# cselab/smarties

Measured on AMD Instinct MI355X. Metric: learner transitions/sec, VRACER batch=256 over 1M replay, higher is better.
Workload: dtype f32; 1 GPU; VRACER learner update, synthetic replay 5000 episodes x 200 transitions = 1M (state_dim 17, act_dim 6 bounded), 2x256 SoftSign MLP (72976 padded fp32 params), global batch 256 split over 1 replica(s), replay split likewise, device-side mt19937 sampler; global_batch=256, replay_transitions=1000000, parallelism=dp1, exchange=single replica

## Files before the change

smarties_amd/csrc/fused.hip:

```cpp
#include "tail_dev.h"

namespace hl {

#define FLDR 258
#define FLDS 34
#define FMAXK4 8
#ifndef FUSED_NT
#define FUSED_NT 512
#endif
#ifndef FUSED_CHAINW
#define FUSED_CHAINW 8
#endif
#ifndef FUSED_PRE_LATE
#define FUSED_PRE_LATE 1
#endif
#ifndef FUSED_H1_PRE
#define FUSED_H1_PRE 1
#endif
#ifndef FUSED_ARGS_FIRST
#define FUSED_ARGS_FIRST 1
#endif
#define FTLD 17

#if defined(HL_FSTAMPS)
// ... 13 lines not shown
#define FEND(i) do { } while (0)
#endif

#ifdef HL_DEV
#define FVARIANT_STOP(n) do { if (a.variant == (n)) return; } while (0)
#else
#define FVARIANT_STOP(n) do { } while (0)
#endif

__host__ __device__ inline int fusedR2Floats(int dSp, int H) { return dSp * (H + 16); }
__host__ __device__ inline int fusedR3Floats(int H) { const int a = H * 16, b = 16 * FLDR; return a > b ? a : b; }
__host__ __device__ inline size_t fusedLdsBytes(int dS, int H) {
  const int dSp = (dS + 3) & ~3;
  const size_t fl = (size_t)16 * FLDR + fusedR2Floats(dSp, H) + fusedR3Floats(H) + (size_t)H * 8  + 16 * FLDS +
                    2048  + 3 * (size_t)H  + 512  + 128  + 2 * (16 * FTLD + 16)  + 32  + 4 ;
  const size_t bytes = fl * 4;
  return bytes > TAIL_LDS_BYTES ? bytes : TAIL_LDS_BYTES;
}

template <int NK, class FA, class FB>
__device__ __forceinline__ f32x4 waveMma(FA fa, FB fb) {
  float av[NK], bv[NK];
#pragma unroll
  for (int s = 0; s < NK; ++s) { av[s] = fa(s); bv[s] = fb(s); }
  f32x4 acc0 = {0.f, 0.f, 0.f, 0.f}, acc1 = {0.f, 0.f, 0.f, 0.f};
#pragma unroll
  for (int s = 0; s < NK; ++s) {
    if (s & 1) acc1 = __builtin_amdgcn_mfma_f32_16x16x4f32(av[s], bv[s], acc1, 0, 0, 0);
    else acc0 = __builtin_amdgcn_mfma_f32_16x16x4f32(av[s], bv[s], acc0, 0, 0, 0);
  }
  return acc0 + acc1;
}

template <int NQ, int NTL, bool TILE_A, class FS, class FT>
__device__ __forceinline__ void h1Steps(f32x4* acc, FS fs, FT ft) {
  float sv[NQ], tv[NQ][NTL];
#pragma unroll
  for (int s = 0; s < NQ; ++s) {
    sv[s] = fs(s);
#pragma unroll
    for (int t = 0; t < NTL; ++t) tv[s][t] = ft(s, t);
  }
  __builtin_amdgcn_sched_barrier(0);
#pragma unroll
  for (int s = 0; s < NQ; ++s) {
#pragma unroll
    for (int t = 0; t < NTL; ++t) {
      if constexpr (TILE_A) acc[t] = __builtin_amdgcn_mfma_f32_16x16x4f32(tv[s][t], sv[s], acc[t], 0, 0, 0);
      else acc[t] = __builtin_amdgcn_mfma_f32_16x16x4f32(sv[s], tv[s][t], acc[t], 0, 0, 0);
    }
  }
}
template <int NTL, bool TILE_A, class FS, class FT>
__device__ __forceinline__ void h1Product(int nk4, f32x4* acc, FS fs, FT ft) {
  switch (nk4) {
    case 1: h1Steps<1, NTL, TILE_A>(acc, fs, ft); break;
    case 2: h1Steps<2, NTL, TILE_A>(acc, fs, ft); break;
    case 3: h1Steps<3, NTL, TILE_A>(acc, fs, ft); break;
    case 4: h1Steps<4, NTL, TILE_A>(acc, fs, ft); break;
    case 5: h1Steps<5, NTL, TILE_A>(acc, fs, ft); break;
    case 6: h1Steps<6, NTL, TILE_A>(acc, fs, ft); break;
    case 7: h1Steps<7, NTL, TILE_A>(acc, fs, ft); break;
    case 8: h1Steps<8, NTL, TILE_A>(acc, fs, ft); break;
    default: break;
  }
}

template <int NP> __device__ __forceinline__ float redSum(const float* red, int tid) {
  if constexpr (NP == 8) return ((red[tid] + red[256 + tid]) + (red[512 + tid] + red[768 + tid])) + ((red[1024 + tid] + red[1280 + tid]) + (red[1536 + tid] + red[1792 + tid]));
  else return (red[tid] + red[256 + tid]) + (red[512 + tid] + red[768 + tid]);
}

template <int N> __device__ __forceinline__ float treeSum(const float* v) {
  if constexpr (N == 1) return v[0];
  else return treeSum<N / 2>(v) + treeSum<N / 2>(v + N / 2);
}

template <int H, int CF, int NT>
__global__ __launch_bounds__(NT, NT / 128) void fused_fwd_head_dx_kernel(FusedArgs a, ExtraArgs extra) {
  extern __shared__ __attribute__((aligned(16))) unsigned char smem[];
  if (blockIdx.x < 8) {
    if (threadIdx.x >= 256) return;
    if (blockIdx.x == 0) { if (extra.role == 1) { samplePhases(extra.samp, extra.phases, smem); FEND(22); } }
    else if (blockIdx.x == 1 && (a.deferBeta || extra.post.mode == POST_ENCODE)) { farBetaPhase(extra.post, smem); if (threadIdx.x == 0) a.sc->dbgT[23] = wall_clock64(); }
    else if (extra.role == 1 && (extra.phases & PH_PUBLISH)) gatherHelper(extra.samp, blockIdx.x - 1, 7, smem);
    return;
  }
  constexpr int HT = H / 16, H4 = H / 4, LDW0 = H + 16;
  constexpr int NW = NT / 64;
  constexpr int KWAVES = (H / 4 >= NW) ? NW : 4;
  constexpr int KW = H / KWAVES;
  constexpr int NK = KW / 4;
  constexpr int TPW = HT >= NW ? HT / NW : 1;
  constexpr int QP = (16 * H4 + NT - 1) / NT;
  constexpr int QC = (H * 4 + NT - 1) / NT;
  constexpr int QO = (H * 2 + NT - 1) / NT;
  constexpr int Q0 = (32 * H4 + NT - 1) / NT;
  constexpr int QS = 512 / NT;
  constexpr bool CHAIN = (NW == 8 && H >= 64);
  constexpr int CW = (FUSED_CHAINW == 8 && H >= 128) ? 8 : 4;
  constexpr int CT = CHAIN ? H / (16 * CW) : 1;
  constexpr int CTID = CW == 8 ? 0 : 256;
  constexpr int TLD = CHAIN ? FTLD : 16;
  constexpr int TY1 = 16 * FTLD + 16;
#if defined(HL_FSTAMPS)
  if (threadIdx.x == 0 && blockIdx.x == 8 + 8) a.sc->dbgT[31] = wall_clock64();
#endif
#ifdef HL_TAIL_STAMPS
  if (threadIdx.x == 0 && blockIdx.x == 8 + 8) a.sc->dbgT[31] = wall_clock64();
#endif
#ifdef HL_STEP_STAMPS
  if (threadIdx.x == 0 && blockIdx.x == 8 + 8) a.sc->dbgStep[a.sc->nGradSteps & 63] = wall_clock64();
#endif
  const DevScalars* sc = a.sc;
  const float* W = a.W; const float* X0 = a.X0; unsigned* panelCtr = a.panelCtr;
  long long iW0 = a.indW0, iW1 = a.indW1, iWo = a.indWo, iB0 = a.indB0, iB1 = a.indB1, iWr = a.indWr, iBr = a.indBr, iBo = a.indBo, iBp = a.indBp;
  int ldW0 = a.ldW0, ldW1 = a.ldW1, ldX0 = a.ldX0, dSa = a.dS, Ba = a.B, parity = a.parity;
#if FUSED_ARGS_FIRST
  asm volatile("" :: "s"(W), "s"(iW0), "s"(iW1), "s"(iWo), "s"(iB0), "s"(iB1), "s"(iWr), "s"(iBr), "s"(iBo), "s"(iBp),
               "s"(X0), "s"(panelCtr), "s"(sc), "s"(ldW0), "s"(ldW1), "s"(ldX0), "s"(dSa), "s"(Ba), "s"(parity),
               "s"(a.bt.nextSrc), "s"(a.bt.slot), "s"(a.bt.eid));
#endif
  const int dS = dSa, dSp = (dS + 3) & ~3, B = Ba, dA = a.dA, nDense = a.nDense;
  const int func = __builtin_amdgcn_readfirstlane(a.func);
  int resN = a.resN, ldA0 = a.ldA0, ldA1 = a.ldA1;
  float* gR2 = a.R2; float* gX2 = a.X2; float* gD2 = a.D2; float* gDres2 = a.Dres2;
#define FUSED_PIN_ARGS() do { asm volatile("" : "+v"(resN), "+v"(ldA0), "+v"(ldA1)); asm volatile("" : "+v"(gR2), "+v"(gX2), "+v"(gD2), "+v"(gDres2)); } while (0)
#if !FUSED_ARGS_FIRST
  FUSED_PIN_ARGS();
#endif
  const int bid = blockIdx.x - 8, xcd = bid & 7, gi = bid >> 3;
  const int panel = (gi / HT) * 8 + xcd, n = gi % HT;
  const int m0 = panel * 16, n0 = n * 16;
  int nRows = B;
  if (m0 + 16 > B) { nRows = sc->nRows[parity]; if (m0 >= nRows) return; }
  FSTAMP(0);

  float* sY1 = reinterpret_cast<float*>(smem);
  float* sR2 = sY1 + 16 * FLDR;
  float* sR3 = sR2 + fusedR2Floats(dSp, H);
  float* sWo = sR3 + fusedR3Floats(H);
  float* sS = sWo + H * 8;
  float* red = sS + 16 * FLDS;
  float* sB0 = red + 2048;
  float* sWr = sB0 + H;
  float* sBr = sWr + H;
  double* sO = reinterpret_cast<double*>(sBr + H);
  float* sDo = reinterpret_cast<float*>(sO + 256);
  float* sT = sDo + 128;
  float* sBo = sT + 2 * (16 * FTLD + 16);
  float* sBp = sBo + 16;
  double* sBeta = reinterpret_cast<double*>(sBp + 16);

  const int tid = threadIdx.x, lane = tid & 63;
  __builtin_assume(tid >= 0 && tid < NT);
  const int wave = __builtin_amdgcn_readfirstlane(tid >> 6);
  const int li = lane & 15, lc = lane >> 4;
  const bool eth = tid < 256;
  const int em = (tid >> 4) & 15, en = tid & 15;
  const float* W0 = W + iW0; const float* W1 = W + iW1; const float* Wo = W + iWo;

  const int row = m0 + em;
  const bool rowValid = eth && row < nRows, isNext = rowValid && row >= B;
  int bSrc = 0; long long slot = 0;
  if (rowValid) { bSrc = isNext ? a.bt.nextSrc[row - B] : row; slot = a.bt.slot[bSrc]; }
  int eidv = 0;
  if (rowValid && !isNext) eidv = a.bt.eid[row];
  float sv[QS];
#pragma unroll
  for (int q = 0; q < QS; ++q) {
    const int idx = tid + NT * q, r = idx >> 5, c = idx & 31;
    sv[q] = (c < dS && m0 + r < nRows) ? X0[(size_t)(m0 + r) * ldX0 + c] : 0.f;
  }
  const f32x4 z4 = {0.f, 0.f, 0.f, 0.f};
  f32x4 w0v[Q0], w1c[QC], w1r[QP], wov[QO];
  const int nW0 = dSp * H4;
#pragma unroll
  for (int q = 0; q < Q0; ++q) {
    const int f = tid + NT * q, k = f / H4, c4 = f % H4;
    w0v[q] = *reinterpret_cast<const f32x4*>(W0 + (size_t)(k < dS ? k : dS - 1) * ldW0 + 4 * c4);
  }
#pragma unroll
  for (int q = 0; q < QC; ++q) {
    const int f = tid + NT * q; w1c[q] = z4;
    if (f < H * 4) { const int k = f >> 2, c = n0 + (f & 3) * 4; w1c[q] = *reinterpret_cast<const f32x4*>(W1 + (size_t)k * ldW1 + c); }
  }
#pragma unroll
  for (int q = 0; q < QO; ++q) { const int f = tid + NT * q; wov[q] = f < H * 2 ? *reinterpret_cast<const f32x4*>(Wo + (size_t)f * 4) : z4; }
  const float b0v = tid < H ? W[iB0 + tid] : 0.f;
  const float wrv = tid < H ? W[iWr + tid] : 0.f, brv = tid < H ? W[iBr + tid] : 0.f;
  const float b1e = eth ? W[iB1 + n0 + en] : 0.f;
  const float bov = tid < nDense ? W[iBo + tid] : 0.f, bpv = tid < dA ? W[iBp + tid] : 0.f;
  double beta = sc->beta; const double Cmax = sc->Cmax, Cinv = sc->Cinv;
  const long long betaWant = sc->nGradSteps;
  unsigned ctr0 = 0;
  if constexpr (HT > 1) ctr0 = __hip_atomic_load(panelCtr + panel * 32, __ATOMIC_RELAXED, __HIP_MEMORY_SCOPE_AGENT);
#if FUSED_ARGS_FIRST
  FUSED_PIN_ARGS();
#endif
#pragma unroll
  for (int q = 0; q < QS; ++q) { const int idx = tid + NT * q, r = idx >> 5, c = idx & 31; sS[r * FLDS + c] = sv[q]; }
#pragma unroll
  for (int q = 0; q < Q0; ++q) {
    const int f = tid + NT * q;
    if (f < nW0) { const int k = f / H4, c4 = f % H4; *reinterpret_cast<f32x4*>(sR2 + k * LDW0 + 4 * c4) = w0v[q]; }
  }
#pragma unroll
  for (int q = 0; q < QC; ++q) { const int f = tid + NT * q; if (f < H * 4) *reinterpret_cast<f32x4*>(sR3 + (size_t)f * 4) = w1c[q]; }
#pragma unroll
  for (int q = 0; q < QO; ++q) { const int f = tid + NT * q; if (f < H * 2) *reinterpret_cast<f32x4*>(sWo + (size_t)f * 4) = wov[q]; }
  if (tid < H) { sB0[tid] = b0v; sWr[tid] = wrv; sBr[tid] = brv; }
  if (tid < 16) { sBo[tid] = bov; sBp[tid] = bpv; }
  __syncthreads();
  FSTAMP(1);
  FVARIANT_STOP(1);
#pragma unroll
  for (int q = 0; q < QP; ++q) {
    const int f = tid + NT * q; w1r[q] = z4;
    if (f < 16 * H4) { const int r = f / H4, c4 = f % H4; w1r[q] = *reinterpret_cast<const f32x4*>(W1 + (size_t)(n0 + r) * a.ldW1 + 4 * c4); }
  }
  const bool aggOwner = ((em & (HT - 1)) == n) && rowValid && !isNext && en < AGG_N;

  double act = 0, bMean = 0, bStd = 1; float misc = 0.f;
  if (rowValid && !isNext && en < dA) {
    act = a.rp.A[(size_t)slot * dA + en];
    bMean = a.rp.MU[(size_t)slot * 2 * dA + en]; bStd = a.rp.MU[(size_t)slot * 2 * dA + dA + en];
  }
  if (rowValid) {
    const float* arr = nullptr; long long sl = slot;
    if (!isNext) arr = en == 0 ? a.rp.RET : en == 1 ? a.rp.DQ : en == 2 ? a.rp.DKL : en == 3 ? a.rp.IMPW : en == 4 ? a.rp.V : en == 5 ? a.rp.ADV : nullptr;
    else { arr = en == 6 ? a.rp.V : en == 7 ? a.rp.ADV : nullptr; sl = slot + 1; }
    if (arr) misc = arr[sl];
  }

  float aggv = 0.f;
  if constexpr (CHAIN) {
    asm volatile("" : "+v"(eidv));
    if (aggOwner) aggv = en < AGG_USED ? a.rp.epAgg[(size_t)eidv * AGG_N + en] : (en == AGG_LEN ? (float)a.rp.epN[eidv] : 0.f);
  }

  const bool live = rowValid && !isNext;
  const double MAXM = 8.31776613503286;
  double stdev = 1, invStd = 1, dPos = 0, bInv = 1, invVarMu = 1, u2 = 0, lq = 0, CmuCpi = 1;
  bool bnd = false;
  auto headPrecompute = [&]() {
    asm volatile("" : "+v"(act), "+v"(bMean), "+v"(bStd));
    if (live && en < dA) {
      bnd = ((a.boundedMask >> en) & 1ull) != 0;
      const double pp = (double)sBp[en];
      const double rt = sqrt(1 + pp * pp);
      stdev = (pp + rt) / 2; invStd = 1 / stdev; dPos = (1 + pp / rt) / 2;
      bInv = 1 / bStd; invVarMu = 1 / (bStd * bStd);
      u2 = (act - bMean) * bInv;
      const double qq = stdev * bInv;
      lq = log(qq); CmuCpi = qq * qq;
    }
  };

  float x1o = 0.f, y1o = 0.f;
  if constexpr (!CHAIN) {
  if (wave < HT) {
    f32x4 acc[TPW];
#pragma unroll
    for (int t = 0; t < TPW; ++t) acc[t] = z4;
    const int nk4 = dSp >> 2;
    float bb[TPW];
#pragma unroll
    for (int t = 0; t < TPW; ++t) bb[t] = sB0[(wave + NW * t) * 16 + li];
#if FUSED_H1_PRE
    h1Product<TPW, false>(nk4, acc, [&](int s) { return sS[li * FLDS + 4 * s + lc]; },
                          [&](int s, int t) { return sR2[(4 * s + lc) * LDW0 + (wave + NW * t) * 16 + li]; });
#else
    float av = sS[li * FLDS + lc], bv[TPW];
#pragma unroll
    for (int t = 0; t < TPW; ++t) bv[t] = sR2[lc * LDW0 + (wave + NW * t) * 16 + li];
    for (int s = 0; s < nk4; ++s) {
      const int kn = s + 1 < nk4 ? 4 * (s + 1) + lc : lc;
      const float avn = sS[li * FLDS + kn];
      float bvn[TPW];
#pragma unroll
      for (int t = 0; t < TPW; ++t) bvn[t] = sR2[kn * LDW0 + (wave + NW * t) * 16 + li];
#pragma unroll
      for (int t = 0; t < TPW; ++t) acc[t] = __builtin_amdgcn_mfma_f32_16x16x4f32(av, bv[t], acc[t], 0, 0, 0);
      av = avn;
#pragma unroll
      for (int t = 0; t < TPW; ++t) bv[t] = bvn[t];
    }
#endif
    FSTAMP(14);
    dispatchFunc<CF>(func, [&](auto F) {
      constexpr int FN = decltype(F)::value;
#pragma unroll
      for (int t = 0; t < TPW; ++t) {
        const int nt = wave + NW * t;
        const int c = nt * 16 + li;
#pragma unroll
        for (int r = 0; r < 4; ++r) {
          const int i = lc * 4 + r;
          const float x = acc[t][r] + bb[t];
          sY1[i * FLDR + c] = actEvalT<FN>(x);
          if (nt == n) sT[i * 16 + li] = x;
        }
      }
    });
  }
  FSTAMP(15);
  __syncthreads();
  x1o = sT[em * 16 + en]; y1o = sY1[em * FLDR + n0 + en];
  FSTAMP(2);
  FVARIANT_STOP(2);
  if (eth && row < B) a.Y1[(size_t)row * ldA0 + n0 + en] = y1o;
  asm volatile("" : "+v"(eidv));
  if (aggOwner) aggv = en < AGG_USED ? a.rp.epAgg[(size_t)eidv * AGG_N + en] : (en == AGG_LEN ? (float)a.rp.epN[eidv] : 0.f);
  }
  constexpr bool SPLITW = (NW == 8 && H >= 16);
  constexpr int XW = CHAIN ? CW : (SPLITW ? 4 : KWAVES);
  constexpr int XKW = H / XW, XNK = XKW / 4;

  if constexpr (CHAIN) {
    const int cw = CW == 8 ? wave : wave - 4;
    if (cw >= 0) {
      const int cb = cw * XKW;
      const int pc = (li >> 2) + 4 * (li & 3);
      float w1b[CT][4];
#pragma unroll
      for (int t = 0; t < CT; ++t) {
#pragma unroll
        for (int r = 0; r < 4; ++r) w1b[t][r] = sR3[(cb + 16 * t + 4 * r + lc) * 16 + li];
      }
      f32x4 acc[CT];
#pragma unroll
      for (int t = 0; t < CT; ++t) acc[t] = z4;
      const int nk4 = dSp >> 2;
      float bb[CT][4];
#pragma unroll
      for (int t = 0; t < CT; ++t) {
#pragma unroll
        for (int r = 0; r < 4; ++r) bb[t][r] = sB0[cb + 16 * t + 4 * r + lc];
      }
#if FUSED_H1_PRE
      h1Product<CT, true>(nk4, acc, [&](int s) { return sS[li * FLDS + 4 * s + lc]; },
                          [&](int s, int t) { return sR2[(4 * s + lc) * LDW0 + cb + 16 * t + pc]; });
#else
      float bv = sS[li * FLDS + lc], av[CT];
#pragma unroll
      for (int t = 0; t < CT; ++t) av[t] = sR2[lc * LDW0 + cb + 16 * t + pc];
      for (int s = 0; s < nk4; ++s) {
        const int kn = s + 1 < nk4 ? 4 * (s + 1) + lc : lc;
        const float bvn = sS[li * FLDS + kn];
        float avn[CT];
#pragma unroll
        for (int t = 0; t < CT; ++t) avn[t] = sR2[kn * LDW0 + cb + 16 * t + pc];
#pragma unroll
        for (int t = 0; t < CT; ++t) acc[t] = __builtin_amdgcn_mfma_f32_16x16x4f32(av[t], bv, acc[t], 0, 0, 0);
        bv = bvn;
#pragma unroll
        for (int t = 0; t < CT; ++t) av[t] = avn[t];
      }
#endif
      FSTAMPT(CTID, 14);
      dispatchFunc<CF>(func, [&](auto F) {
        constexpr int FN = decltype(F)::value;
#pragma unroll
        for (int t = 0; t < CT; ++t) {
          const bool own = cb + 16 * t == n0;
#pragma unroll
          for (int r = 0; r < 4; ++r) {
            const float x = acc[t][r] + bb[t][r], y = actEvalT<FN>(x);
            acc[t][r] = y;
            if (own) { sT[li * TLD + 4 * r + lc] = x; sT[TY1 + li * TLD + 4 * r + lc] = y; }
          }
        }
      });
      FSTAMPT(CTID, 15);
      f32x4 xa0 = z4, xa1 = z4;
#pragma unroll
      for (int t = 0; t < CT; ++t) {
#pragma unroll
        for (int r = 0; r < 4; ++r) {
          if (r & 1) xa1 = __builtin_amdgcn_mfma_f32_16x16x4f32(acc[t][r], w1b[t][r], xa1, 0, 0, 0);
          else xa0 = __builtin_amdgcn_mfma_f32_16x16x4f32(acc[t][r], w1b[t][r], xa0, 0, 0, 0);
        }
      }
      const f32x4 xacc = xa0 + xa1;
#pragma unroll
      for (int r = 0; r < 4; ++r) red[cw * 256 + (lc * 4 + r) * 16 + li] = xacc[r];
      FSTAMPT(CTID, 16);
      if (CW == 8 && !FUSED_PRE_LATE) headPrecompute();
    } else if (!FUSED_PRE_LATE) headPrecompute();
    FSTAMP(2);
    FVARIANT_STOP(2);
  } else {
    const int xw = SPLITW ? wave - 4 : wave;
    if (xw >= 0 && xw < XW) {
      const int k0 = xw * XKW + lc;
      const f32x4 acc = waveMma<XNK>([&](int s) { return sY1[li * FLDR + k0 + 4 * s]; }, [&](int s) { return sR3[(k0 + 4 * s) * 16 + li]; });
// ... 187 lines not shown
    const double g0 = far ? 0.0 : Ver * beta * scaleVdiff(O0);
    const double coef = A_RET * fmin(Cmax, RHO);
    if (live && en < dA) {
      const double dMean = mean - bMean;
      const double penalM = -1 * (dMean * invVarMu);
      const double penalS = dPos * -1 * ((invVarMu - invStd * invStd) * stdev);
      double polM = 0, polS = 0;
      if (!far) {
        if (bnd) {
          const double dLogPdMean = (act - mean) * invStd * invStd;
          const double m = mean > MAXM ? MAXM : (mean < -MAXM ? -MAXM : mean);
          const double u = (act - m) * invStd;
          polS = dPos * coef * ((u * u - 1) * invStd);
          if (mean >= MAXM && coef * dLogPdMean > 0) polM = 0;
          else if (mean <= -MAXM && coef * dLogPdMean < 0) polM = 0;
          else polM = coef * dLogPdMean;
        } else {
          const double u = (act - mean) * invStd;
          polM = coef * (u * invStd);
          polS = dPos * coef * ((u * u - 1) * invStd);
        }
      }
      const double gM = beta * polM + (1 - beta) * penalM;
      const double gS = beta * polS + (1 - beta) * penalS;
      gMf = (float)gM;
      if (writer) {
        a.bt.gParam[(size_t)bSrc * dA + en] = (float)gS;
        a.bt.G[(size_t)bSrc * a.nOut + 1 + en] = (double)gMf;
        a.bt.G[(size_t)bSrc * a.nOut + nDense + en] = (double)(float)gS;
      }
    }
    if (live) g0f = (float)g0;
    const float gPrev = rowRorF<1>(gMf);
    if (en < 8) sDo[em * 8 + en] = en == 0 ? g0f : (en <= dA ? gPrev : 0.f);
    if (live && writer) {
      const float oDQ = rowRorF<15>(misc), oDKL = rowRorF<14>(misc), oW = rowRorF<13>(misc);
      const float oV = rowRorF<12>(misc), oADV = rowRorF<11>(misc);
      if (en == 0) {
        a.bt.pEid[bSrc] = a.bt.eid[bSrc]; a.bt.pNextOf[bSrc] = a.bt.nextOf[bSrc];
        a.bt.G[(size_t)bSrc * a.nOut] = (double)g0f;
        a.bt.rho[bSrc] = RHO; a.bt.dkl[bSrc] = DKL; a.bt.far[bSrc] = far ? 1 : 0;
        const float E = (float)dQ, D = (float)DKL, Wn = (float)RHO, Vf = (float)V;
        a.bt.oldDQ[bSrc] = oDQ; a.bt.oldDKL[bSrc] = oDKL; a.bt.oldW[bSrc] = oW; a.bt.oldV[bSrc] = oV; a.bt.oldADV[bSrc] = oADV;
        a.bt.newDQ[bSrc] = E; a.bt.newDKL[bSrc] = D; a.bt.newW[bSrc] = Wn; a.bt.newV[bSrc] = Vf;
        a.rp.DQ[slot] = E; a.rp.DKL[slot] = D; a.rp.IMPW[slot] = Wn; a.rp.V[slot] = Vf; a.rp.ADV[slot] = 0.f;
        a.bt.dq[bSrc] = (double)E;
      }
      if (en < nDense) a.bt.O[(size_t)row * a.nOut + en] = (double)Oen;
      if (en < dA) a.bt.O[(size_t)row * a.nOut + nDense + en] = (double)sBp[en];
    }
  }
  if (NW != 8) stageF2();
  __syncthreads();
  FSTAMP(10);
  FVARIANT_STOP(7);
  if (eth && writer && row < B && en < nDense) a.dOut[(size_t)row * a.ldDo + en] = sDo[em * 8 + en];

  auto deltaY3 = [&](int rowL, int c) {
    const f32x4 wa = *reinterpret_cast<const f32x4*>(sWo + c * 8), wb = *reinterpret_cast<const f32x4*>(sWo + c * 8 + 4);
    const f32x4 da = *reinterpret_cast<const f32x4*>(sDo + rowL * 8), db = *reinterpret_cast<const f32x4*>(sDo + rowL * 8 + 4);
    float s = wa[0] * da[0];
    s = fmaf(wa[1], da[1], s); s = fmaf(wa[2], da[2], s); s = fmaf(wa[3], da[3], s);
    s = fmaf(wb[0], db[0], s); s = fmaf(wb[1], db[1], s); s = fmaf(wb[2], db[2], s); s = fmaf(wb[3], db[3], s);
    return s;
  };
  float dy3own = 0.f;
  if (eth && rowValid) {
    const int c = n0 + en;
    dy3own = deltaY3(em, c);
    if (row < B) { gDres2[(size_t)row * ldA1 + c] = dy3own; gD2[(size_t)row * ldA1 + c] = dy3own * sF2[em * FLDR + c]; }
  }
  FSTAMP(11);
  FVARIANT_STOP(8);

  if (wave < KWAVES) {
    const int k0 = wave * KW + lc;
    const f32x4 acc = waveMma<NK>([&](int s) { const int c = k0 + 4 * s; return deltaY3(li, c) * sF2[li * FLDR + c]; },
                                  [&](int s) { return sBx[li * FLDR + k0 + 4 * s]; });
#pragma unroll
    for (int r = 0; r < 4; ++r) red[wave * 256 + (lc * 4 + r) * 16 + li] = acc[r];
  }
  __syncthreads();
  FSTAMP(12);
  if (((em & (HT - 1)) == n) && rowValid && !isNext && en < AGG_N) a.bt.aggIn[(size_t)bSrc * AGG_N + en] = aggv;
  if (eth && row < B) {
    const float v = redSum<KWAVES>(red, tid);
    float dres = v;
    if (n0 + en < resN) dres += dy3own * sWr[n0 + en];
    a.Dres1[(size_t)row * ldA0 + n0 + en] = dres;
    float f1 = 1.f;
    dispatchFunc<CF>(func, [&](auto F) { f1 = actDiffT<decltype(F)::value>(x1o, y1o); });
    a.D1[(size_t)row * ldA0 + n0 + en] = dres * f1;
  }
  FSTAMP(13);
  FEND(m0 + 16 > a.B ? 21 : 20);
}

template <int H, int CF>
static hipError_t launchFusedT(const FusedArgs& a, int maxRows, const ExtraArgs& ex, hipStream_t s) {
  const int HT = H / 16, panels = (maxRows + 15) / 16, pg = (panels + 7) / 8;
  const size_t lds = fusedLdsBytes(a.dS, H);
  { hipError_t e = ensureDynLds(reinterpret_cast<const void*>(fused_fwd_head_dx_kernel<H, CF, FUSED_NT>), lds); if (e != hipSuccess) return e; }
  hipLaunchKernelGGL((fused_fwd_head_dx_kernel<H, CF, FUSED_NT>), dim3(8 + 8 * HT * pg), dim3(FUSED_NT), lds, s, a, ex);
  return hipGetLastError();
}
template <int H>
static hipError_t launchFusedH(const FusedArgs& a, int maxRows, const ExtraArgs& ex, hipStream_t s) {
  if (a.func == HL_FUNC_SOFTSIGN) return launchFusedT<H, HL_FUNC_SOFTSIGN>(a, maxRows, ex, s);
  if (a.func == HL_FUNC_TANH) return launchFusedT<H, HL_FUNC_TANH>(a, maxRows, ex, s);
  return launchFusedT<H, -1>(a, maxRows, ex, s);
}

hipError_t launch_fused(const FusedArgs& a, int maxRows, const ExtraArgs* extra, hipStream_t s) {
  ExtraArgs ex{}; if (extra) ex = *extra;
  switch (a.H) {
    case 16: return launchFusedH<16>(a, maxRows, ex, s);
    case 32: return launchFusedH<32>(a, maxRows, ex, s);
    case 64: return launchFusedH<64>(a, maxRows, ex, s);
    case 128: return launchFusedH<128>(a, maxRows, ex, s);
    case 256: return launchFusedH<256>(a, maxRows, ex, s);
    default: return hipErrorInvalidValue;
  }
}

size_t fused_lds_bytes(int dS, int H) { return fusedLdsBytes(dS, H); }
int fused_threads() { return FUSED_NT; }

__global__ void xcc_probe_kernel(int* out) {
  extern __shared__ __attribute__((aligned(16))) unsigned char probeSmem[];
  if (threadIdx.x == 0) out[blockIdx.x] = (int)(__builtin_amdgcn_s_getreg((4 - 1) << 11 | 0 << 6 | 20) & 15);
}
hipError_t launch_xcc_probe(int nBlocks, int nThreads, size_t ldsBytes, int* out, hipStream_t s) {
  { hipError_t e = ensureDynLds(reinterpret_cast<const void*>(xcc_probe_kernel), ldsBytes); if (e != hipSuccess) return e; }
  hipLaunchKernelGGL(xcc_probe_kernel, dim3(nBlocks), dim3(nThreads), ldsBytes, s, out);
  return hipGetLastError();
}

}
```

smarties_amd/csrc/fusedw.hip:

```cpp
#include "head_rows.h"

namespace hl {

#define WLDR 258
constexpr int FW_NT = 512;
constexpr int FW_MAXNT = 5;

#ifdef HL_PANEL_STAMPS
#define WSTMP(i) do { if (threadIdx.x == 0 && panel == 0 && n == 1) scw->dbgT[i] = wall_clock64(); } while (0)
#else
#define WSTMP(i) do { } while (0)
#endif

struct FwGeo { int dSp, LS, NTo, LD, LO; size_t oR2, oR3, oWo, oS, oRed, oVec, oO, oXo, oDelta, oMisc, oAct, oBeta, oT, oY4, oF3, oBx2, oW2c, oVec2, total; };
__host__ __device__ inline FwGeo fwGeo(int dS, int H, int nDense, int nOut, int ldWo, int nAdv, int nLH = 2) {
  FwGeo g;
  g.dSp = (dS + 3) & ~3; g.LS = g.dSp + 2;
  g.NTo = (nDense + 15) / 16; g.LD = g.NTo * 16 + 6; g.LO = nOut | 1;
  size_t o = (size_t)16 * WLDR * 4;
  g.oR2 = o; { size_t a = (size_t)g.dSp * 16 * 4, b = (size_t)16 * WLDR * 4, c = nAdv ? (size_t)2 * 16 * 64 * 8 : 0; if (b > a) a = b; if (c > a) a = c; o += a; }
  g.oR3 = o; { size_t a = (size_t)H * 16 * 4, b = (size_t)16 * WLDR * 4; o += a > b ? a : b; }
  g.oWo = o; o += (size_t)H * ldWo * 4;
  g.oS = o; o += (size_t)16 * g.LS * 4;
  g.oRed = o; o += (size_t)8 * g.NTo * 256 * 4;
  g.oVec = o; o += (size_t)3 * H * 4;
  g.oO = (o + 7) & ~(size_t)7; o = g.oO + (size_t)16 * g.LO * 8;
  g.oXo = o; o += (size_t)16 * g.LD * 4;
  g.oDelta = o; o += (size_t)16 * g.LD * 4;
  g.oMisc = o; o += 16 * 8 * 4;
  g.oAct = (o + 7) & ~(size_t)7; o = g.oAct + 16 * 8;
  g.oBeta = o; o += 16;
  g.oT = o; o += 256 * 4;
  g.oY4 = g.oF3 = g.oBx2 = g.oW2c = g.oVec2 = o;
  if (nLH == 3) {
    g.oY4 = o; o += (size_t)16 * WLDR * 4; g.oF3 = o; o += (size_t)16 * WLDR * 4; g.oBx2 = o; o += (size_t)16 * WLDR * 4;
    g.oW2c = o; o += (size_t)H * 16 * 4; g.oVec2 = o; o += (size_t)2 * H * 4;
  }
  g.total = o > (size_t)TAIL_LDS_BYTES ? o : (size_t)TAIL_LDS_BYTES;
  return g;
}

template <int NP> __device__ __forceinline__ float fwRedSum(const float* red, int tid) {
  if constexpr (NP == 8) return ((red[tid] + red[256 + tid]) + (red[512 + tid] + red[768 + tid])) + ((red[1024 + tid] + red[1280 + tid]) + (red[1536 + tid] + red[1792 + tid]));
  else return (red[tid] + red[256 + tid]) + (red[512 + tid] + red[768 + tid]);
}

template <int NK, class FA, class FB>
__device__ __forceinline__ f32x4 fwWaveMma(FA fa, FB fb) {
  float av[NK], bv[NK];
#pragma unroll
  for (int s = 0; s < NK; ++s) { av[s] = fa(s); bv[s] = fb(s); }
  f32x4 acc0 = {0.f, 0.f, 0.f, 0.f}, acc1 = {0.f, 0.f, 0.f, 0.f};
#pragma unroll
  for (int s = 0; s < NK; ++s) {
    if (s & 1) acc1 = __builtin_amdgcn_mfma_f32_16x16x4f32(av[s], bv[s], acc1, 0, 0, 0);
    else acc0 = __builtin_amdgcn_mfma_f32_16x16x4f32(av[s], bv[s], acc0, 0, 0, 0);
  }
  return acc0 + acc1;
}

template <int H, int NCH, int NLH>
__global__ __launch_bounds__(FW_NT, 2) void fused_wide_kernel(FusedArgs a, HeadArgs ha, ExtraArgs extra) {
  extern __shared__ __attribute__((aligned(16))) unsigned char smem[];
  if (blockIdx.x < 8) {
    if (threadIdx.x >= 256) return;
    if (blockIdx.x == 0) { if (extra.role == 1) samplePhases(extra.samp, extra.phases, smem); }
    else if (blockIdx.x == 1 && (a.deferBeta || extra.post.mode == POST_ENCODE)) farBetaPhase(extra.post, smem);
    return;
  }
  constexpr int NT = FW_NT, NW = NT / 64, HT = H / 16, H4 = H / 4;
  constexpr int KW = H / NW, NK = KW / 4;
  constexpr int QP = (16 * H4 + NT - 1) / NT;
  constexpr int QC = (H * 4 + NT - 1) / NT;
  const DevScalars* sc = a.sc;
  DevScalars* scw = a.sc;
  const int dS = a.dS, B = a.B, dA = a.dA, nDense = a.nDense, nOut = a.nOut, ldWo = ha.ldWo, nSig = ha.nSig;
  const FwGeo g = fwGeo(dS, H, nDense, nOut, ldWo, ha.nAdv, NLH);
  const int dSp = g.dSp, LS = g.LS, NTo = g.NTo, LD = g.LD, LO = g.LO;
  const int func = __builtin_amdgcn_readfirstlane(a.func);
  int resN = a.resN, ldA0 = a.ldA0, ldA1 = a.ldA1;
  asm volatile("" : "+v"(resN), "+v"(ldA0), "+v"(ldA1));
  float* gR2 = a.R2; float* gX2 = a.X2; float* gD2 = a.D2; float* gDres2 = a.Dres2;
  asm volatile("" : "+v"(gR2), "+v"(gX2), "+v"(gD2), "+v"(gDres2));
  const int bid = blockIdx.x - 8, xcd = bid & 7, gi = bid >> 3;
  const int panel = (gi / HT) * 8 + xcd, n = gi % HT;
  const int m0 = panel * 16, n0 = n * 16;
  int nRows = a.B;
  if (m0 + 16 > a.B) { nRows = sc->nRows[a.parity]; if (m0 >= nRows) return; }

  WSTMP(0);
  float* sY1 = reinterpret_cast<float*>(smem);
  float* sR2 = reinterpret_cast<float*>(smem + g.oR2);
  float* sR3 = reinterpret_cast<float*>(smem + g.oR3);
  float* sWo = reinterpret_cast<float*>(smem + g.oWo);
  float* sS = reinterpret_cast<float*>(smem + g.oS);
  float* red = reinterpret_cast<float*>(smem + g.oRed);
  float* sB0 = reinterpret_cast<float*>(smem + g.oVec);
  float* sWr = sB0 + H; float* sBr = sWr + H;
  double* sO = reinterpret_cast<double*>(smem + g.oO);
  float* sXo = reinterpret_cast<float*>(smem + g.oXo);
  float* sDelta = reinterpret_cast<float*>(smem + g.oDelta);
  float* sMisc = reinterpret_cast<float*>(smem + g.oMisc);
  double* sAct = reinterpret_cast<double*>(smem + g.oAct);
  double* sBeta = reinterpret_cast<double*>(smem + g.oBeta);
  float* sT = reinterpret_cast<float*>(smem + g.oT);
  double* sTq = reinterpret_cast<double*>(sR2);
  double* sTr = sTq + 16 * 64;
  float* sY4 = reinterpret_cast<float*>(smem + g.oY4);
  float* sF3 = reinterpret_cast<float*>(smem + g.oF3);
  float* sBx2 = reinterpret_cast<float*>(smem + g.oBx2);
  float* sW2c = reinterpret_cast<float*>(smem + g.oW2c);
  float* sWr2 = reinterpret_cast<float*>(smem + g.oVec2); float* sBr2 = sWr2 + H;

  const int tid = threadIdx.x, lane = tid & 63;
  __builtin_assume(tid >= 0 && tid < NT);
  const int wave = __builtin_amdgcn_readfirstlane(tid >> 6);
  const int li = lane & 15, lc = lane >> 4;
  const bool eth = tid < 256;
  const int em = (tid >> 4) & 15, en = tid & 15;
  const float* W = a.W;
  const float* W0 = W + a.indW0; const float* W1 = W + a.indW1;

  const int row = m0 + em;
  const bool rowValid = eth && row < nRows, isNext = rowValid && row >= B, live = rowValid && !isNext;
  int bSrc = 0; long long slot = 0;
  if (rowValid) { bSrc = isNext ? a.bt.nextSrc[row - B] : row; slot = a.bt.slot[bSrc]; }
  const f32x4 z4 = {0.f, 0.f, 0.f, 0.f};
  const int d4 = dSp >> 2;
  f32x4 sv[4];
  {
    const int r = tid >> 5;
    const float* xr = a.X0 + (size_t)(m0 + r) * a.ldX0;
#pragma unroll
    for (int u = 0; u < 4; ++u) { const int c4 = (tid & 31) + 32 * u; sv[u] = (c4 < d4 && m0 + r < nRows) ? *reinterpret_cast<const f32x4*>(xr + 4 * c4) : z4; }
  }
  constexpr int QW0 = 4;
  f32x4 w0v[QW0], w1c[QC], w1r[QP];
#pragma unroll
  for (int q = 0; q < QW0; ++q) {
    const int f = tid + NT * q, k = f >> 2, c = n0 + (f & 3) * 4;
    w0v[q] = (k < dS) ? *reinterpret_cast<const f32x4*>(W0 + (size_t)k * a.ldW0 + c) : z4;
  }
#pragma unroll
  for (int q = 0; q < QC; ++q) {
    const int f = tid + NT * q; w1c[q] = z4;
    if (f < H * 4) { const int k = f >> 2, c = n0 + (f & 3) * 4; w1c[q] = *reinterpret_cast<const f32x4*>(W1 + (size_t)k * a.ldW1 + c); }
  }
  {
    const f32x4* src = reinterpret_cast<const f32x4*>(W + a.indWo); f32x4* dst = reinterpret_cast<f32x4*>(sWo);
    const int total4 = (H * ldWo) >> 2;
// ... 430 lines not shown
```

smarties_amd/csrc/hl_types.h:

```cpp
#pragma once
#include <stdint.h>
#include "../../include/smarties_hip.h"

namespace hl {

struct DevScalars {
  double beta, alpha, Cmax, Cinv;
  double adam_bt1, adam_bt2;
  double maxAbsErrEMA;
  long long nStep;
  long long nGradSteps;
  long long nFarTotal;
  long long nFarStat;
  long long nTransitions;
  long long nEpisodes;
  long long cnt[4];
  long long seenLocal[2];
  float rewMean, rewScale, rewStd;
  float maxAbsErrAll;
  float maxAbsErrStep;
  unsigned maxAbsScratch;
  int nNext[2];
  int nRows[2];
  float etaEff[2];
  int errFlag;
  long long gatherFlag[2];
  unsigned rngPos;
  unsigned rng[624];
  unsigned rngBakPos;
  unsigned rngBak[624];
  long long seenUpd[2];
  long long sampleSeq;
  double sumRetErr; long long cntRetUpd;
  long long betaSeq;
  unsigned notifySeq;
  long long dbgT[32];
  long long dbgStep[128];
  long long cntPrev[4];
};

struct PosRec {
  long long prefix;
  long long off;
  long long tag;
  int N;
  int eidTerm;
};

constexpr int FAR_REGS = 24, FAR_SUB = 4, FAR_Q = FAR_REGS / FAR_SUB;

struct DevReplay {
  float* S;
  double* A;
  double* MU;
  double* R;
  float *V, *ADV, *RET;
  float *DQ, *IMPW, *DKL;
  long long* epOff;
  int* epN;
  unsigned char* epTerm;
  long long* epTag;
  float* epAgg;
  int* posEid;
  long long* posPrefix;
  struct PosRec* posRec;
  float* stMean; float* stScale; float* stStd;
  float* farP; float* farN; unsigned long long* farStart;
};
enum { AGG_TOTR = 0, AGG_AVGKL, AGG_FRACFAR, AGG_AVGSQERR, AGG_MAXABSERR, AGG_SUMQ2, AGG_SUMQ,
       AGG_MAXQ, AGG_MINQ, AGG_USED, AGG_LEN = 9 , AGG_N = 12 };

struct DevBatch {
  long long* flat;
  int* pos;
  int* eid;
  int* t;
  long long* slot;
  int* nextOf;
  int* nextSrc;
  long long* tag;
  unsigned* sVals;
  int *pEid, *pNextOf;
  double* O;
  double* G;
  double *rho, *dkl, *dq;
  unsigned char* far;
  float *newDQ, *newDKL, *newW, *newV;
  float* newQ;
  float *oldDQ, *oldDKL, *oldW, *oldV, *oldADV;
  float *nextV, *oldNextV, *oldNextADV;
  float* gParam;
  float* aggIn;
};

struct DevHidden {
  int nIn, size, ldW;
  int func;
  long long indW, indB;
  int hasRes, resW;
  int lstm;
  long long indWr, indBr;
  float *X, *Y, *Rr;
  float *D, *Dres;
  int ldA;
};

enum { GEMM_F = 0,
       GEMM_X = 1,
       GEMM_W = 2,
       RED_COL = 3 };
enum { EPI_FWD = 0, EPI_DX = 1, EPI_DW = 2, EPI_NONE = 3 };

struct GemmProblem {
  int flavor, epi;
  int M, N, K;
  int dynRows;
  const float* A; int lda;
  const float* B; int ldb;
  float* C; int ldc;
  const float* bias;
  float* C2; float* C3;
  const float* resW; const float* resB; const float* resIn; int ldRes; int resN;
  const float* actX; const float* actY; int ldAct; int func;
  float* biasOut;
  int adam;
  float *adW, *adM1, *adM2;
  float *adbW, *adbM1, *adbM2;
  int tileStart, tilesM, tilesN;
  int nSplit, adamRed;
  float* part;
  int bigChunk;
};

constexpr int BIG_DW_MAX = 12;
struct BigDwList { int n; int idx[BIG_DW_MAX]; int start[BIG_DW_MAX + 1]; };

struct alignas(128) XchgCtl {
  unsigned long long seq; unsigned long long pad0[15];
  unsigned int done; unsigned int arrived;  unsigned int pad1[30];
};
struct PushArgs {
  int on, nRanks, rank;
  unsigned char* const* peers;
  unsigned long long slotsOffset, slotBytes;
  const XchgCtl* ctl;
  const float* gBase;
};
struct AdamHyper { float eta0, lambda, fac; double epsAnneal; int parity;
                   int variant;
                   PushArgs push; };

}
```

smarties_amd/csrc/kernels.h:

```cpp
#pragma once
#include <hip/hip_runtime.h>
#include <map>
#include <mutex>
#include <string>
#include <utility>
#include "hl_types.h"

namespace hl {

inline hipError_t ensureDynLds(const void* kernel, size_t bytes) {
  static std::mutex m; static std::map<std::pair<int, const void*>, size_t> done;
  int dev = 0; (void)hipGetDevice(&dev);
  std::lock_guard<std::mutex> g(m);
  size_t& have = done[std::make_pair(dev, kernel)];
  if (bytes <= have) return hipSuccess;
  hipError_t e = hipFuncSetAttribute(kernel, hipFuncAttributeMaxDynamicSharedMemorySize, (int)bytes);
  if (e == hipSuccess) have = bytes;
  return e;
}

struct SampleArgs {
  DevScalars* sc; DevReplay rp; DevBatch bt;
  int B, dS, ldX0;
  float* X0;
// ... 60 lines not shown
};
constexpr int TM_WIN_MAX_IN = 8192;
enum { TM_PART_PREPARE = 1, TM_PART_PRODUCT = 2, TM_PART_CHAIN = 4, TM_PART_ALL = 7 };
struct WinRowsArgs { const DevScalars* sc; DevScalars* scW; const long long* slot; const int* t; const int* nextSrc; int B, K, nBPTT, parity;
                     long long* slotW; int* tW; int* nextSrcW; };
hipError_t launch_window_rows(const WinRowsArgs& a, hipStream_t s);
hipError_t launch_rec_forward(const RecArgs& a, hipStream_t s);
hipError_t launch_rec_backward(const RecArgs& a, hipStream_t s);
bool rec_tm_ok(const RecArgs& a);
bool rec_tm_act_ok(const RecArgs& a);
bool rec_win_act_ok(const RecArgs& a);
std::string rec_route_name(const RecArgs& a, bool backward);
hipError_t launch_rec_tm_forward(const RecArgs& a, hipStream_t s, int parts = TM_PART_ALL);
hipError_t launch_rec_tm_backward(const RecArgs& a, hipStream_t s);
struct ExtraArgs;
bool rec_step_fused_ok(const RecArgs& a, const HeadArgs& ha);
hipError_t launch_rec_step_fused(const RecArgs& a, const HeadArgs& ha, const ExtraArgs* extra, hipStream_t s);

struct ConvGeo {
  int InC, InY, InX, KnC, KnY, KnX, S, OpY, OpX;
  int K, P;
  int ldIn, ldOut;
  long long indW, indB;
  const float* in;
  float* X; float* Y;
  float* D;
  float* part;
  float* Wf; float* Wx;
  int nChunks, chunkRows, dwBlock0;
  int rbRows, rbCount, rbWin;
  int rbKind;
  int dwG;
};
struct ConvSource {
  int on;
  const float* S; const float* mean; const float* scale; int dS, nApp;
  const long long* slot; const int* t; const int* nextSrc;
};
struct ConvArgs {
  DevScalars* sc; int parity, B, nL;
  const float* W; float* Wrw; float* M1; float* M2; float* G;
  ConvGeo L[HL_MAX_CONV];
  ConvSource src;
};
struct StackGatherArgs { DevScalars* sc; DevReplay rp; DevBatch bt; int B, dS, nApp, parity; float* X0; int ldX0; };
struct AdamHyper;
hipError_t launch_stack_gather(const StackGatherArgs& a, int maxRows, hipStream_t s);
hipError_t launch_extras_copy(const DevScalars* sc, int parity, const float* X0, int ldX0, int col0, int n, float* dst, int ldDst, int maxRows, hipStream_t s);
hipError_t launch_conv_prep(const ConvArgs& a, hipStream_t s);
long long conv_prep_floats(const ConvGeo& g, int which);
hipError_t launch_conv_forward(const ConvArgs& a, int l, int maxRows, hipStream_t s);
struct GemmProblem;
struct DenseRide { const GemmProblem* probs; int nProbs, tile0, tile1, own; AdamHyper hyp; };
hipError_t launch_conv_dx(const ConvArgs& a, int l, hipStream_t s, const DenseRide* ride = nullptr);
bool conv_dx_rides(const ConvGeo& g);
hipError_t launch_conv_dw(const ConvArgs& a, int totalBlocks, hipStream_t s);
int conv_row_block(const ConvGeo& g, int* win);
int conv_dw_staged_group(const ConvGeo& g, int B);
bool conv_rows_atari(const ConvGeo& g, const ConvSource& src);
bool conv_rows_ok(const ConvGeo& g);
hipError_t launch_conv_forward_rows(const ConvArgs& a, int l, int maxRows, hipStream_t s);
hipError_t launch_conv_dw_all(const ConvArgs& a, int l, int dwBlocks, hipStream_t s);
hipError_t launch_conv_dw_rows(const ConvArgs& a, int l, hipStream_t s);
hipError_t launch_conv_reduce_adam(const ConvArgs& a, const AdamHyper& hyp, int fuseAdam, hipStream_t s);

struct ConvTailPlan {
  int on;
  int icPer[HL_MAX_CONV];
  int bufD;
  int ldsBack;
  int atari;
};
bool conv_tail_plan(const ConvGeo* L, int nL, ConvTailPlan* pl);
hipError_t launch_conv_back(const ConvArgs& a, const ConvTailPlan& pl, hipStream_t s);
hipError_t launch_conv_fwd_tail(const ConvArgs& a, const ConvTailPlan& pl, int maxRows, hipStream_t s);

struct PostArgs {
  DevScalars* sc; DevReplay rp; DevBatch bt;
  int B, mode;
  double clipImpWeight, epsAnneal, penalTol, maxObsGlobal, batchGlobal;
  int nRanks;
  int parity;
  float eta0;
  int aggStaged;
  int hasAdv;
  int aggChunk;
  float* cntMsg;
  int behind;
};
enum { POST_AGG = 1, POST_BETA = 2, POST_INIT = 4, POST_ENCODE = 8 ,
       POST_DEFER = 16 ,
       POST_KEEPMSG = 32  };

struct AdamArgs {
  const DevScalars* sc; float* W; float* M1; float* M2; const float* G; long long n;
  float eta0, lambda, fac; double epsAnneal; int parity;
};

constexpr int XCHG_CHUNKS = 64;
constexpr int XCHG_CHUNKS_NODE = 32;
constexpr int XCHG_MAX_RANKS = 16;
struct XchgArgs {
  void* msg; long long n;
  int nRanks, rank;
  unsigned char* const* peers;
  size_t slotsOffset, slotBytes;
  XchgCtl* ctl; DevScalars* sc;
  long long timeoutTicks;
  int fuse; AdamArgs adam; PostArgs post;
  long long pushed;
  int maxChunks;
};
int xchg_chunks(long long bytes, int maxChunks);
hipError_t launch_xchg_allreduce(const XchgArgs& a, int dtype , hipStream_t s);
hipError_t launch_xchg_clean(unsigned char* win, size_t slotsOffset, size_t slotBytes, int nRanks, const XchgCtl* ctl, long long bytes, hipStream_t s);
enum { PH_A = 1, PH_B = 2, PH_C = 4, PH_ALL = 7, PH_PUBLISH = 8 };
struct ExtraArgs { int role; int phases; SampleArgs samp; PostArgs post; int helpers;  };
hipError_t launch_conv_dw_dense(const ConvArgs& a, int l, int dwBlocks, const GemmProblem* dProbs, int nProbs, int nTiles, const AdamHyper& hyp,
                                const ExtraArgs* extra, hipStream_t s);

struct FusedArgs {
  DevScalars* sc; DevReplay rp; DevBatch bt;
  int B, dS, dA, nDense, nOut, H, parity, func, resN;
  const float* X0; int ldX0;
  const float* W;
  long long indW0, indB0, indW1, indB1, indWr, indBr, indWo, indBo, indBp; int ldW0, ldW1;
  float* Y1; float* D1; float* Dres1; int ldA0;
  float* X2; float* R2; float* D2; float* Dres2; int ldA1;
  int nLH; long long indW2, indB2, indWr2, indBr2; int ldW2, resN2;
  float* X3; float* R3; float* D3; float* Dres3; int ldA2;
  float* dOut; int ldDo;
  unsigned* panelCtr;
  float* Opart;
  int variant;
  int deferBeta;
  int xcdSafe;
  unsigned long long boundedMask;
};

struct EpisodeSweepArgs {
  DevScalars* sc; DevReplay rp;
  const int* eids; int count;
  float gamma, lambda; int recompute;
  int skipRetrace;
  float* redMaxAbs;
  int retKind;
  double* redErr;
};

struct MomentsArgs {
  DevScalars* sc; DevReplay rp; int dS; int nEpisodes;
  double* partial; int nBlocks;
  double* moments;
  int bInit; double learnrate, epsAnneal, rRateFac;
};

bool big_panel_ok(const GemmProblem& P);
hipError_t launch_big_panel(const GemmProblem& P, const DevScalars* sc, int parity, hipStream_t s);
bool big_mm_ok(const GemmProblem& P);
hipError_t launch_big_mm(const GemmProblem& P, const DevScalars* sc, int parity, hipStream_t s);
bool big_dw_ok(const GemmProblem& P);
int big_dw_chunk_rows(const GemmProblem& P);
int big_dw_blocks(const GemmProblem& P);
hipError_t launch_big_dw(const GemmProblem* dProbs, const BigDwList& L, hipStream_t s);
bool panel_head_ok(const HeadArgs& a);
hipError_t launch_panel_head(const HeadArgs& a, int maxRows, const ExtraArgs* extra, hipStream_t s);
hipError_t launch_sample(const SampleArgs& a, hipStream_t s);
hipError_t launch_post_agg_chunks(const PostArgs& a, hipStream_t s);
hipError_t launch_step_tail(const PostArgs* post, const SampleArgs* samp, hipStream_t s, int phases = PH_ALL);
enum { GEMM_ROLE_FWD0 = 0, GEMM_ROLE_FWD = 1, GEMM_ROLE_DX = 2, GEMM_ROLE_DW = 3 };
constexpr int DW_TABLE_MAX = 8;
struct DwTable { GemmProblem p[DW_TABLE_MAX]; int n; };
hipError_t launch_dw_table(const DwTable& tbl, int nBlocks, const DevScalars* sc, const AdamHyper& hyp, const ExtraArgs* extra, hipStream_t s,
                           const ExtraArgs* extra2 = nullptr);
hipError_t launch_gemm(int role, const GemmProblem* dProbs, int nProbs, int nBlocks, const DevScalars* sc,
// ... 143 lines not shown
```

smarties_amd/csrc/learner.cpp:

```cpp
#include <hip/hip_runtime.h>
#include <rccl/rccl.h>

#include <algorithm>
#include <array>
#include <cfloat>
#include <cmath>
#include <cstdio>
#include <cstdlib>
#include <chrono>
#include <atomic>
#include <unistd.h>
#include <cstring>
#include <deque>
#include <map>
#include <mutex>
#include <string>
#include <sstream>
#include <iomanip>
#include <climits>
#include <limits>
#include <vector>

#include "kernels.h"

// ... 223 lines not shown
      const int HT = h->hid[1].size / 16, panels = (h->Mmax + 15) / 16, pg = (panels + 7) / 8, nBlk = 8 + 8 * HT * pg;
      int* dX = nullptr; HIPCK(devAlloc(&dX, (size_t)nBlk));
      HIPCK(launch_xcc_probe(nBlk, fused_threads(), fused_lds_bytes(h->dS, h->hid[1].size), dX, h->stream));
      std::vector<int> xcc((size_t)nBlk);
      HIPCK(hipMemcpyAsync(xcc.data(), dX, xcc.size() * sizeof(int), hipMemcpyDeviceToHost, h->stream));
      HIPCK(hipStreamSynchronize(h->stream)); hipFree(dX);
      bool same = true;
      for (int b = 8; b < nBlk; ++b) same = same && xcc[(size_t)b] == xcc[(size_t)(8 + ((b - 8) & 7))];
      const char* f = getenv("SMARTIES_HIP_PANEL_SAFE");
      h->xcdSafe = !same || (f && f[0] == '1');
      const size_t nCtr = (size_t)roundUp((h->Mmax + 15) / 16, 8) * 32;
      HIPCK(devAlloc(&h->panelCtr, nCtr));
      HIPCK(hipMemset(h->panelCtr, 0, nCtr * sizeof(unsigned)));
      HIPCK(devAlloc(&h->panelOpart, (nCtr / 32) * (size_t)HT * 128));
      HIPCK(hipStreamSynchronize(nullptr));
    }
  }
  if (!h->fusedOk && (h->nHidden == 2 || h->nHidden == 3) && !h->recurrent && !h->preproc && !(h->generic & 1)) {
    const DevHidden& d0 = h->hid[0]; const DevHidden& d1 = h->hid[1];
    const int comps = h->nOpt ? h->nOpt : h->dA, nLH = h->nHidden;
    bool ok = d0.size == d1.size && !d0.hasRes && d1.hasRes && d1.nIn == d0.size && d0.func == d1.func &&
              fused_wide_ok(h->dS, d1.size, h->nDense, h->nOut, h->ldWo, cfg->adv_kind == HL_ADV_GAUSSIAN ? h->nAdv : 0, comps, nLH);
    if (nLH == 3) { const DevHidden& d2 = h->hid[2]; ok = ok && d2.size == d1.size && d2.hasRes && d2.nIn == d1.size && d2.func == d1.func && !(h->generic & 512); }
    if (ok) {
      const int HT = d1.size / 16, panels = (h->Mmax + 15) / 16, pg = (panels + 7) / 8, nBlk = 8 + 8 * HT * pg;
      int* dX = nullptr; HIPCK(devAlloc(&dX, (size_t)nBlk));
      HIPCK(launch_xcc_probe(nBlk, fused_wide_threads(), fused_wide_lds_bytes(h->dS, d1.size, h->nDense, h->nOut, h->ldWo, cfg->adv_kind == HL_ADV_GAUSSIAN ? h->nAdv : 0, nLH), dX, h->stream));
      std::vector<int> xcc((size_t)nBlk);
      HIPCK(hipMemcpyAsync(xcc.data(), dX, xcc.size() * sizeof(int), hipMemcpyDeviceToHost, h->stream));
      HIPCK(hipStreamSynchronize(h->stream)); hipFree(dX);
      for (int b = 8; b < nBlk; ++b) ok = ok && xcc[(size_t)b] == xcc[(size_t)(8 + ((b - 8) & 7))];
      const char* f = getenv("SMARTIES_HIP_PANEL_SAFE");
      ok = ok && !(f && f[0] == '1');
    }
    if (ok) {
      const size_t nCtr = (size_t)roundUp((h->Mmax + 15) / 16, 8) * 32;
      HIPCK(devAlloc(&h->panelCtr, nCtr));
      h->fusedWideOk = true;
    }
  }
  h->noDeferBeta = (h->generic & 2) != 0;
  h->noConvReplay = (h->generic & 64) != 0;
  if (!h->fusedOk && !h->fusedWideOk && !h->recurrent && !h->bigBatch) {
    const int j0 = h->nConv > 0 ? 1 : 0;
    bool ok = h->nHidden - j0 >= 2 && !(h->generic & 2);
    int HT = 0;
    for (int j = j0; j < h->nHidden; ++j) { ok = ok && !gemm_oneshot_ok(GEMM_F, h->hid[j].nIn); HT = std::max(HT, (h->hid[j].size + 15) / 16); }
    ok = ok && HT <= 64;
    if (ok) {
      const int nBlk = fwd_chain_blocks(h->Mmax, HT);
      int* dX = nullptr; HIPCK(devAlloc(&dX, (size_t)nBlk));
      HIPCK(launch_xcc_probe(nBlk, 256, fwd_chain_lds_bytes(), dX, h->stream));
      std::vector<int> xcc((size_t)nBlk);
      HIPCK(hipMemcpyAsync(xcc.data(), dX, xcc.size() * sizeof(int), hipMemcpyDeviceToHost, h->stream));
      HIPCK(hipStreamSynchronize(h->stream)); hipFree(dX);
      for (int b = 8; b < nBlk; ++b) ok = ok && xcc[(size_t)b] == xcc[(size_t)(8 + ((b - 8) & 7))];
      const char* f = getenv("SMARTIES_HIP_PANEL_SAFE");
      ok = ok && !(f && f[0] == '1');
    }
    if (ok) {
      const size_t nCtr = (size_t)roundUp((h->Mmax + 15) / 16, 8) * 32;
      HIPCK(devAlloc(&h->panelCtr, nCtr));
      h->chainOk = true; h->chainHT = HT;
      bool sc = h->nConv == 0 && !(h->generic & 512) && HT <= 32;
      for (int j = 1; j < h->nHidden; ++j) sc = sc && !gemm_oneshot_ok(GEMM_X, h->hid[j].size);
      h->stepChainOk = sc;
    }
  }
  h->ldDo = (int)roundUp(h->nDense, 16);
  HIPCK(devAlloc(&h->dOut, (size_t)B * h->ldDo));
  for (int pb = 0; pb < 2; ++pb) {
    DevBatch& bt = h->buf[pb].bt;
    HIPCK(devAlloc(&h->buf[pb].X0, (size_t)h->convMmax * h->ldX0));
    HIPCK(devAlloc(&bt.flat, B)); HIPCK(devAlloc(&bt.pos, B)); HIPCK(devAlloc(&bt.eid, B)); HIPCK(devAlloc(&bt.t, B));
    HIPCK(devAlloc(&bt.slot, B)); HIPCK(devAlloc(&bt.nextOf, B)); HIPCK(devAlloc(&bt.nextSrc, B));
    HIPCK(devAlloc(&bt.tag, B)); HIPCK(devAlloc(&bt.pEid, B)); HIPCK(devAlloc(&bt.pNextOf, B));
    HIPCK(devAlloc(&bt.sVals, (size_t)std::max(B, 256)));
    HIPCK(devAlloc(&bt.O, (size_t)2 * B * h->nOut)); HIPCK(devAlloc(&bt.G, (size_t)B * h->nOut));
    HIPCK(devAlloc(&bt.rho, B)); HIPCK(devAlloc(&bt.dkl, B)); HIPCK(devAlloc(&bt.dq, B)); HIPCK(devAlloc(&bt.far, B));
    HIPCK(devAlloc(&bt.newDQ, B)); HIPCK(devAlloc(&bt.newDKL, B)); HIPCK(devAlloc(&bt.newW, B)); HIPCK(devAlloc(&bt.newV, B)); HIPCK(devAlloc(&bt.newQ, B));
    HIPCK(devAlloc(&bt.oldDQ, B)); HIPCK(devAlloc(&bt.oldDKL, B)); HIPCK(devAlloc(&bt.oldW, B)); HIPCK(devAlloc(&bt.oldV, B));
    HIPCK(devAlloc(&bt.oldADV, B)); HIPCK(devAlloc(&bt.nextV, B)); HIPCK(devAlloc(&bt.oldNextV, B));
    HIPCK(devAlloc(&bt.oldNextADV, B)); HIPCK(devAlloc(&bt.gParam, (size_t)B * std::max(h->nSig, 1)));
    HIPCK(devAlloc(&bt.aggIn, (size_t)B * AGG_N));
  }
  HIPCK(devAlloc(&h->dFlatGiven, B));
  HIPCK(devAlloc(&h->dMoments, (size_t)2 * h->dS + 3)); HIPCK(devAlloc(&h->dMomentsPrev, (size_t)2 * h->dS + 3)); HIPCK(devAlloc(&h->dStatsOut, 16)); HIPCK(devAlloc(&h->dStatsIns, 16));
  HIPCK(devAlloc(&h->rp.stMean, h->dS)); HIPCK(devAlloc(&h->rp.stScale, h->dS)); HIPCK(devAlloc(&h->rp.stStd, h->dS));
  HIPCK(devAlloc(&h->rp.farStart, 4 * 256));
  {
    const long long slack = std::max<long long>(512, std::min<long long>(8192, (64ll << 20) / ((long long)h->dS * 4)));
    rc = growSlots(h, h->maxObsLocal + h->maxObsLocal / 8 + slack); if (rc) return rc;
  }
  rc = growEpisodes(h, 4096); if (rc) return rc;
  DevScalars s0; std::memset(&s0, 0, sizeof(s0));
  s0.beta = cfg->clipImpWeight <= 0 ? 1 : 1e-4; s0.alpha = 0.5;
  s0.Cmax = 1 + cfg->clipImpWeight; s0.Cinv = 1 / cfg->clipImpWeight;
  s0.adam_bt1 = 0.9; s0.adam_bt2 = 0.999; s0.rewMean = 0; s0.rewScale = 1; s0.rewStd = 1;
  s0.cntRetUpd = cfg->returnsEstimator == HL_RET_NONE ? -1 : 0;
  { HostMT g; uint32_t sd = (uint32_t)(cfg->randSeed + (uint64_t)cfg->rank); g.x[0] = sd;
    for (uint32_t i = 1; i < 624; ++i) g.x[i] = 1812433253u * (g.x[i - 1] ^ (g.x[i - 1] >> 30)) + i;
    g.p = 624;
    for (int t = 1; t < cfg->ref_threads; ++t) (void)g.next();
    std::memcpy(s0.rng, g.x, sizeof(g.x)); s0.rngPos = g.p; }
  HIPCK(hipMemcpy(h->sc, &s0, sizeof(s0), hipMemcpyHostToDevice));
  std::vector<float> ones(h->dS, 1.f);
  HIPCK(hipMemcpy(h->rp.stScale, ones.data(), h->dS * sizeof(float), hipMemcpyHostToDevice));
  HIPCK(hipMemcpy(h->rp.stStd, ones.data(), h->dS * sizeof(float), hipMemcpyHostToDevice));
  rc = buildProblems(h); if (rc) return rc;
  if (h->wideIn && !rec_tm_ok(recArgs(h, 0))) return fail(h, HL_ERR_UNSUPPORTED, "wide recurrent input: the time-step-major launches refuse this net");
  if (const char* e = getenv("SMARTIES_HIP_NO_GRAPH")) { if (e[0] == '1') h->useGraph = false; }
  if (const char* e = getenv("SMARTIES_HIP_XCHG_TIMEOUT_MS")) h->xchgTimeoutTicks = std::max(1LL, atoll(e)) * 100000LL;
  return HL_OK;
}

int hl_destroy(hl_learner* h) {
  if (!h) return HL_OK;
  h->mu.lock();
  if (h->stream) hipStreamSynchronize(h->stream);
  if (h->sideStream) hipStreamSynchronize(h->sideStream);
  timerFlush(h);
  invalidateGraphs(h);
  if (h->comm) ncclCommDestroy(h->comm);
  for (unsigned char* q : {h->act.pin, h->act.rowsPin, h->act.convPin}) if (q) hipHostFree(q);
  if (h->notifyPin) hipHostFree(h->notifyPin);
  for (void* q : h->xchg.opened) hipIpcCloseMemHandle(q);
  if (h->xchg.win) { windowPoolPut(h->dev, h->xchg.winBytes, h->xchg.win); h->xchg.win = nullptr; }
  for (void* q : {(void*)h->xchg.dPeers, (void*)h->xchg.ctl}) if (q) hipFree(q);
  void* ptrs[] = {h->splitPart, h->widePart, h->wideCtr, h->W, h->M1, h->M2, h->G, h->sc, h->dOut, h->dProbs, h->dFlatGiven, h->dEidList,
    h->dRedMax, h->dRedErr, h->dMomPartial, h->dMoments, h->dMomentsPrev, h->dStatsOut, h->dStatsIns,
    h->rp.S, h->rp.A, h->rp.MU, h->rp.R, h->rp.V, h->rp.ADV, h->rp.RET, h->rp.DQ, h->rp.IMPW, h->rp.DKL,
    h->rp.epOff, h->rp.epN, h->rp.epTerm, h->rp.epAgg, h->rp.posEid, h->rp.posPrefix, h->rp.stMean, h->rp.stScale,
    h->rp.stStd, h->rp.epTag, h->rp.posRec, h->rp.farP, h->rp.farN, h->rp.farStart, h->panelCtr, h->panelOpart, h->act.dS, h->act.dO, h->act.convFeat, h->act.devStamps, h->act.devOut, h->act.devSums, h->act.devRows};
  for (hipEvent_t ev : {h->act.devIn, h->act.devDone}) if (ev) hipEventDestroy(ev);
  for (int pb = 0; pb < 2; ++pb) {
    DevBatch& bt = h->buf[pb].bt;
    void* bp[] = {h->buf[pb].X0, bt.sVals, bt.tag, bt.pEid, bt.pNextOf, bt.flat, bt.pos, bt.eid, bt.t, bt.slot, bt.nextOf, bt.nextSrc,
      bt.O, bt.G, bt.rho, bt.dkl, bt.dq, bt.far, bt.newDQ, bt.newDKL, bt.newW, bt.newV, bt.newQ, bt.oldDQ, bt.oldDKL, bt.oldW,
      bt.oldV, bt.oldADV, bt.nextV, bt.oldNextV, bt.oldNextADV, bt.gParam, bt.aggIn};
    for (void* q : bp) if (q) hipFree(q);
  }
  for (void* q : {(void*)h->segY, (void*)h->segDres, (void*)h->segScratch}) if (q) hipFree(q);
  for (void* q : {(void*)h->winSlot, (void*)h->winT, (void*)h->winNextSrc, (void*)h->scW}) if (q) hipFree(q);
  for (int j = 0; j < HL_MAX_HIDDEN; ++j) for (float* q : {h->rec[j].A, h->rec[j].X, h->rec[j].Y, h->rec[j].D, h->rec[j].Rd, h->rec[j].A2}) if (q) hipFree(q);
  for (int j = 0; j < HL_MAX_HIDDEN; ++j) for (float* q : {h->tmER[j], h->tmSD[j], h->tmFP[j], h->tmET[j]}) if (q) hipFree(q);
  for (void* q : {(void*)h->tmT, (void*)h->tmSteps, (void*)h->tmNext, (void*)h->tmCtr, (void*)h->tmP}) if (q) hipFree(q);
  for (void* p : ptrs) if (p) hipFree(p);
  for (int l = 0; l < h->nConv; ++l) { ConvGeo& g = h->cg[l];
    if (l != h->nConv - 1) for (float* p : {g.X, g.Y, g.D}) if (p) hipFree(p);
    for (float* p : {g.part, g.Wf, g.Wx}) if (p) hipFree(p); }
  for (int j = 0; j < h->nHidden; ++j) { DevHidden& d = h->hid[j];
    for (float* p : {d.X, d.Y, d.Rr, d.D, d.Dres}) if (p) hipFree(p); }
  if (h->pinned) hipHostFree(h->pinned);
  for (auto& st : h->stg) { if (st.host) hipHostFree(st.host); if (st.ev) hipEventDestroy(st.ev); }
  for (void* q : {(void*)h->perProb, (void*)h->perKey, (void*)h->perKeyS, (void*)h->perCp, (void*)h->perIdx, (void*)h->perIdxS, h->perTemp, h->perScan}) if (q) hipFree(q);
  if (h->sideStream) { hipStreamSynchronize(h->sideStream); hipStreamDestroy(h->sideStream); }
  if (h->evMain) hipEventDestroy(h->evMain);
  if (h->evSide) hipEventDestroy(h->evSide);
  if (h->stream) hipStreamDestroy(h->stream);
  h->mu.unlock();
  delete h; return HL_OK;
}

int64_t hl_num_params(const hl_learner* h) { return h ? h->nParams : -1; }
int32_t hl_num_outputs(const hl_learner* h) { return h ? h->nOut : -1; }
int32_t hl_num_layers(const hl_learner* h) { return h ? (int32_t)h->indW.size() : -1; }
int hl_param_layout(const hl_learner* h, int64_t* indW, int64_t* nW, int64_t* indB, int64_t* nB) {
  if (!h) return HL_ERR_BAD_ARG;
  HL_LOCK(h);
  for (size_t l = 0; l < h->indW.size(); ++l) {
    if (indW) indW[l] = h->indW[l];
    if (nW) nW[l] = h->nW[l];
    if (indB) indB[l] = h->indB[l];
    if (nB) nB[l] = h->nB[l];
  }
  return HL_OK;
}

int hl_init_weights(hl_learner* h) {
  if (!h) return HL_ERR_BAD_ARG;
  HL_LOCK(h);
  int rc = dropPresample(h); if (rc) return rc;
  DevScalars s; rc = syncScalarsToHost(h, &s); if (rc) return rc;
  HostMT g; std::memcpy(g.x, s.rng, sizeof(g.x)); g.p = s.rngPos;
  auto uni = [&](float a, float b) {
    float r = (float)g.next() / 4294967296.0f;
    if (r >= 1.0f) r = std::nextafter(1.0f, 0.0f);
    return std::fmaf(r, b - a, a);
  };
  auto initFactor = [&](int f, int inps, int outs) -> double {
    switch (f) { case HL_FUNC_LINEAR: return std::sqrt(1. / inps); case HL_FUNC_TANH: return std::sqrt(6. / (inps + outs));
      case HL_FUNC_SOFTSIGN: return std::sqrt(6.0 / (inps + outs)); case HL_FUNC_RELU: return std::sqrt(2. / inps);
      case HL_FUNC_LRELU: return std::sqrt(1.0 / inps); case HL_FUNC_SIGM: case HL_FUNC_HARDSIGN: return std::sqrt(6. / (inps + outs));
      case HL_FUNC_SOFTPLUS: case HL_FUNC_EXPPLUS: case HL_FUNC_EXP: return std::sqrt(2. / inps); }
    return 1;
  };
  std::vector<float> W((size_t)h->nParams, 0.f);
  for (int l = 0; l < h->nConv; ++l) {
    const ConvGeo& g = h->cg[l];
    const float init = (float)initFactor(HL_FUNC_SOFTSIGN, g.K, g.KnC);
    for (long long w = 0; w < (long long)g.KnC * g.K; ++w) W[g.indW + w] = uni(-init, init);
  }
  for (int j = h->nConv > 0 ? 1 : 0; j < h->nHidden; ++j) {
    const DevHidden& d = h->hid[j];
    const float fac = 1; const float init = fac * initFactor(d.func, d.nIn, d.size);
    if (d.lstm == 1) {
      for (int i = 0; i < d.nIn + d.size; ++i) for (int o = 0; o < d.size; ++o) W[d.indW + o + (long long)d.ldW * i] = uni(-init, init);
    } else if (d.lstm) {
      const int nC = d.size;
      if (d.lstm == 4) for (int o = 0; o < nC; ++o) { W[d.indB + o] = 0.f; W[d.indB + nC + o] = -1.f; W[d.indB + 2 * nC + o] = 1.f; W[d.indB + 3 * nC + o] = -1.f; }
      else for (int o = 0; o < nC; ++o) { W[d.indB + o] = 1.f; W[d.indB + nC + o] = 0.f; }
      for (long long w = 0; w < (long long)d.lstm * nC * (d.nIn + nC); ++w) W[d.indW + w] = uni(-init, init);
    } else
    for (int i = 0; i < d.nIn; ++i) for (int o = 0; o < d.size; ++o) W[d.indW + o + (long long)d.ldW * i] = uni(-init, init);
    if (d.hasRes) for (int o = 0; o < d.size; ++o) { W[d.indWr + o] = 1.f; W[d.indBr + o] = 0.f; }
  }
  { const DevHidden& q = h->hid[h->nHidden - 1];
    const double iFac = h->cfg.outWeightsPrefac; const float fac = (iFac > 0) ? iFac : 1;
    const int oF = h->cfg.nnOutputFunc;
    const float init = fac * initFactor(oF, q.size, h->nDense);
    auto inverse = [&](float in) -> float {
      switch (oF) { case HL_FUNC_TANH: return std::log((1 + in) / (1 - in)) / 2; case HL_FUNC_SIGM: return -std::log(1 / in - 1);
// ... 504 lines not shown
```

smarties_amd/csrc/step_exec.h:

```cpp
#pragma once

namespace {

constexpr int GRAPH_SIZES[] = {999, 256, 128, 64, 32, 16, 8, 4, 2, 1};
constexpr int CNT_MSG_FLOATS = 16;
constexpr int CNT_MSG_OFFSET = 128;
static_assert(CNT_MSG_OFFSET % 4 == 0 && CNT_MSG_FLOATS % 4 == 0, "the counters message is whole 16-byte units (xchgAllreduce)");

void setTiles(GemmProblem& p, int& cursor, bool maySplit = false) {
  p.tilesM = (p.M + 15) / 16; p.tilesN = (p.N + 15) / 16;
  if (p.flavor == RED_COL) { p.tilesM = 1; p.tilesN = (p.N + 15) / 16; }
  p.nSplit = (maySplit && (p.flavor == GEMM_W || p.flavor == RED_COL) && p.K >= 1024) ? (p.K + 255) / 256 : 1;
  p.tileStart = cursor; cursor += p.tilesM * p.tilesN * p.nSplit;
}

int buildProblems(hl_learner* h) {
  std::vector<GemmProblem> P;
  const int nH = h->nHidden, B = h->B;
  for (int pb = 0; pb < 2; ++pb) {
    StepBuf& sb = h->buf[pb];
    sb.fwdIdx.clear(); sb.fwdBlocks.clear(); sb.dxIdx.clear(); sb.dxBlocks.clear(); sb.bigDw.clear();
    const int j0 = h->nConv > 0 ? 1 : 0;
    if (j0) { sb.fwdIdx.push_back(-1); sb.fwdBlocks.push_back(0); }
    for (int j = j0; j < nH && !h->recurrent; ++j) {
// ... 110 lines not shown
      p.C = h->G + h->indWo; p.ldc = h->ldWo; p.biasOut = h->G + h->indBo;
      placeDw(p, h->bigBatch); P.push_back(p);
      if (h->nSig) {
        GemmProblem s{}; s.flavor = RED_COL; s.epi = EPI_NONE; s.N = h->dA; s.K = B;
        s.A = sb.bt.gParam; s.lda = h->dA; s.B = nullptr; s.C = h->G + h->indBp;
        placeDw(s, h->bigBatch); P.push_back(s);
      }
    }
    sb.dwCount = (int)P.size() - sb.dwIdx; sb.dwBlocks = cur;
    {
      size_t need = 0; sb.splitMaxMN = 0;
      for (int i = 0; i < sb.dwCount; ++i) { const GemmProblem& q = P[sb.dwIdx + i]; if (q.nSplit > 1) { const int mn = q.flavor == RED_COL ? q.N : q.M * q.N; need += (size_t)q.nSplit * mn; sb.splitMaxMN = std::max(sb.splitMaxMN, mn); } }
      if (h->wideIn && need > ((size_t)1 << 30)) return fail(h, HL_ERR_UNSUPPORTED, "wide recurrent input: the weight-gradient partials (row chunks x (input + cells + 1) x gates x cells) exceed 2^30 floats");
      if (need > h->splitPartFloats) { if (h->splitPart) hipFree(h->splitPart); h->splitPart = nullptr; HIPCK(devAlloc(&h->splitPart, need)); h->splitPartFloats = need; }
      size_t off = 0;
      for (int i = 0; i < sb.dwCount; ++i) { GemmProblem& q = P[sb.dwIdx + i]; if (q.nSplit > 1) { q.part = h->splitPart + off; off += (size_t)q.nSplit * (q.flavor == RED_COL ? q.N : q.M * q.N); } }
    }
    sb.dwAdamIdx = (int)P.size();
    for (int i = 0; i < sb.dwCount; ++i) {
      GemmProblem p = P[sb.dwIdx + i];
      p.adam = p.nSplit > 1 ? 0 : 1; p.adamRed = p.nSplit > 1 ? 1 : 0;
      const long long offC = p.C - h->G;
      p.adW = h->W + offC; p.adM1 = h->M1 + offC; p.adM2 = h->M2 + offC;
      if (p.biasOut) { const long long offB = p.biasOut - h->G; p.adbW = h->W + offB; p.adbM1 = h->M1 + offB; p.adbM2 = h->M2 + offB; }
      P.push_back(p);
    }
    sb.dwWideIdx = sb.dwWideAdamIdx = -1; sb.dwWideBlocks = 0;
    if (h->recurrent && sb.splitMaxMN > 0) {
      for (int pass = 0; pass < 2; ++pass) {
        (pass ? sb.dwWideAdamIdx : sb.dwWideIdx) = (int)P.size();
        int curW = 0;
        for (int i = 0; i < sb.dwCount; ++i) {
          GemmProblem q = P[(pass ? sb.dwAdamIdx : sb.dwIdx) + i];
          q.nSplit = 1; q.part = nullptr; q.adamRed = 0; q.adam = pass;
          q.tileStart = curW; curW += q.tilesM * q.tilesN;
          P.push_back(q);
        }
        sb.dwWideBlocks = curW;
      }
      if (sb.dwWideBlocks > h->wideTiles) {
        if (h->widePart) hipFree(h->widePart); if (h->wideCtr) hipFree(h->wideCtr);
        h->widePart = nullptr; h->wideCtr = nullptr; h->wideTiles = (int)roundUp(sb.dwWideBlocks, 8);
        HIPCK(devAlloc(&h->widePart, (size_t)h->wideTiles * DW_WIDE_Q * 256));
        HIPCK(devAlloc(&h->wideCtr, (size_t)h->wideTiles));
        HIPCK(hipMemset(h->wideCtr, 0, (size_t)h->wideTiles * sizeof(unsigned)));
      }
    }
    sb.dwTable = DwTable{}; sb.dwTableAdam = DwTable{};
    if (sb.dwCount <= DW_TABLE_MAX) {
      sb.dwTable.n = sb.dwTableAdam.n = sb.dwCount;
      for (int i = 0; i < sb.dwCount; ++i) { sb.dwTable.p[i] = P[sb.dwIdx + i]; sb.dwTableAdam.p[i] = P[sb.dwAdamIdx + i]; }
    }
  }
  if (h->dProbs) hipFree(h->dProbs);
  h->dProbs = nullptr;
  HIPCK(devAlloc(&h->dProbs, P.size()));
  HIPCK(hipMemcpy(h->dProbs, P.data(), P.size() * sizeof(GemmProblem), hipMemcpyHostToDevice));
  h->hostProbs = P;
  return HL_OK;
}

AdamHyper adamHyper(const hl_learner* h, int parity) {
  AdamHyper a{}; a.eta0 = (float)h->cfg.learnrate; a.lambda = (float)h->cfg.nnLambda; a.fac = (float)(1.0 / h->Bglobal);
  a.epsAnneal = h->cfg.epsAnneal; a.parity = parity; a.variant = h->dbgVariant;
  if (h->pushGrad) {
    a.push.on = 1; a.push.nRanks = h->cfg.n_ranks; a.push.rank = h->cfg.rank; a.push.peers = h->xchg.dPeers;
    a.push.slotsOffset = h->xchg.slotsOffset; a.push.slotBytes = h->xchg.slotBytes; a.push.ctl = h->xchg.ctl; a.push.gBase = h->G;
  }
  return a;
}
SampleArgs sampleArgs(hl_learner* h, int parity, const long long* dFlat, bool computeEta) {
  SampleArgs sa{}; sa.sc = h->sc; sa.rp = h->rp; sa.bt = h->buf[parity].bt; sa.B = h->B; sa.dS = h->dS; sa.ldX0 = h->ldX0;
  sa.X0 = h->buf[parity].X0; sa.flatGiven = dFlat; sa.adamDraws = 1;
  sa.parity = parity; sa.computeEta = computeEta ? 1 : 0; sa.backupRng = 0; sa.noGather = (h->preproc || h->recurrent) ? 1 : 0; sa.eta0 = (float)h->cfg.learnrate; sa.epsAnneal = h->cfg.epsAnneal;
  return sa;
}
bool exchanging(const hl_learner* h) { return h->cfg.n_ranks > 1 || h->comm != nullptr; }
bool wired(const hl_learner* h) { return h->comm != nullptr || h->xchg.on; }
bool oneBehind(const hl_learner* h) { return h->xchg.on && h->cfg.n_ranks > 1 && h->cfg.reduction_timing == HL_RDX_ONE_BEHIND; }
PostArgs postArgs(hl_learner* h, int parity, int mode) {
  PostArgs pa{}; pa.sc = h->sc; pa.rp = h->rp; pa.bt = h->buf[parity].bt; pa.B = h->B; pa.mode = mode;
  pa.clipImpWeight = h->cfg.clipImpWeight; pa.epsAnneal = h->cfg.epsAnneal; pa.penalTol = h->cfg.penalTol;
  pa.maxObsGlobal = (double)h->maxObsGlobal; pa.batchGlobal = (double)h->Bglobal; pa.nRanks = exchanging(h) ? 2 : 1;
  pa.parity = parity; pa.eta0 = (float)h->cfg.learnrate; pa.aggStaged = h->fusedOk ? 1 : 0; pa.hasAdv = h->nAdv > 0 ? 1 : 0;
  pa.cntMsg = wired(h) ? h->G + h->nParams + CNT_MSG_OFFSET : nullptr;
  pa.behind = oneBehind(h) ? 1 : 0;
  return pa;
}
HeadArgs headArgs(hl_learner* h, int parity) {
  const DevHidden& q = h->hid[h->nHidden - 1];
  HeadArgs ha{}; ha.sc = h->sc; ha.rp = h->rp; ha.bt = h->buf[parity].bt; ha.B = h->B; ha.dA = h->dA; ha.nDense = h->nDense; ha.nAdv = h->cfg.adv_kind == HL_ADV_GAUSSIAN ? h->nAdv : 0; ha.nOpt = h->nOpt; ha.nSig = h->nSig;
  ha.nOut = h->nOut; ha.H = q.size; ha.Yin = q.hasRes ? q.Rr : q.Y; ha.ldY = q.ldA; ha.Xlast = q.X; ha.Ylast = q.Y;
  ha.func = q.func; ha.params = h->W; ha.indWo = h->indWo; ha.indBo = h->indBo; ha.indBp = h->indBp; ha.ldWo = h->ldWo;
  ha.dOut = h->dOut; ha.ldDo = h->ldDo; ha.Dres = q.Dres; ha.D = q.D; ha.ldD = q.ldA; ha.parity = parity; ha.outFunc = h->cfg.nnOutputFunc;
  for (int i = 0; i < h->dA; ++i) ha.bounded[i] = h->cfg.bounded[i];
  return ha;
}

int launchPerPrepare(hl_learner* h, hipStream_t s) {
  const long long n = std::max<long long>(h->nTransitions, (long long)h->order.size());
  if (n > h->perCap) {
    HIPCK(hipStreamSynchronize(s));
    for (void* q : {(void*)h->perProb, (void*)h->perKey, (void*)h->perKeyS, (void*)h->perCp, (void*)h->perIdx, (void*)h->perIdxS, h->perTemp, h->perScan}) if (q) hipFree(q);
    const size_t cap = (size_t)n + (size_t)n / 4 + 1024;
    HIPCK(devAlloc(&h->perProb, cap)); HIPCK(devAlloc(&h->perCp, cap));
    { h->perScanBytes = per_scan_scratch_bytes((long long)cap); unsigned char* t = nullptr; HIPCK(devAlloc(&t, h->perScanBytes)); h->perScan = t; }
    if (h->cfg.dataSamplingAlgo == HL_SAMPLE_PERRANK) {
      HIPCK(devAlloc(&h->perKey, cap)); HIPCK(devAlloc(&h->perKeyS, cap)); HIPCK(devAlloc(&h->perIdx, cap)); HIPCK(devAlloc(&h->perIdxS, cap));
      h->perTempBytes = per_sort_temp_bytes((long long)cap);
      unsigned char* t = nullptr; HIPCK(devAlloc(&t, h->perTempBytes)); h->perTemp = t;
    }
    h->perCap = (long long)cap;
  }
  PerArgs pa{}; pa.rp = h->rp; pa.nEpisodes = (int)h->order.size(); pa.algo = h->cfg.dataSamplingAlgo;
  pa.prob = h->perProb; pa.cp = h->perCp; pa.key = h->perKey; pa.keySorted = h->perKeyS; pa.idx = h->perIdx; pa.idxSorted = h->perIdxS;
  pa.temp = h->perTemp; pa.tempBytes = h->perTempBytes;
  pa.scan = h->perScan; pa.scanBytes = h->perScanBytes;
  HIPCK(timed(h, "per_prepare", s, [&] { return launch_per_prepare(pa, h->nTransitions, s); }));
  return HL_OK;
}
int launchSample(hl_learner* h, int parity, const long long* dFlat, bool computeEta, hipStream_t s) {
  SampleArgs sa = sampleArgs(h, parity, dFlat, computeEta);
  if (h->cfg.dataSamplingAlgo != HL_SAMPLE_UNIFORM && !dFlat) {
    int rc = launchPerPrepare(h, s); if (rc) return rc;
    sa.perAlgo = h->cfg.dataSamplingAlgo; sa.perCp = h->perCp;
    sa.perN = h->cfg.dataSamplingAlgo == HL_SAMPLE_PERSEQ ? (long long)h->order.size() : h->nTransitions;
  }
  HIPCK(timed(h, "step_tail_kernel", s, [&] { return launch_sample(sa, s); }));
  return HL_OK;
}
ExtraArgs extraSample(hl_learner* h, int parityNext, int phases) {
  ExtraArgs ex{}; ex.role = 1; ex.phases = phases; ex.samp = sampleArgs(h, parityNext, nullptr, false);
  ex.samp.backupRng = 1;
  return ex;
}
FusedArgs fusedArgs(hl_learner* h, int parity) {
  const DevHidden& d0 = h->hid[0]; const DevHidden& d1 = h->hid[1];
  FusedArgs fa{}; fa.sc = h->sc; fa.rp = h->rp; fa.bt = h->buf[parity].bt;
  fa.B = h->B; fa.dS = h->dS; fa.dA = h->dA; fa.nDense = h->nDense; fa.nOut = h->nOut; fa.H = d1.size; fa.parity = parity;
  fa.func = d1.func; fa.resN = d1.resW;
  fa.X0 = h->buf[parity].X0; fa.ldX0 = h->ldX0; fa.W = h->W;
  fa.indW0 = d0.indW; fa.indB0 = d0.indB; fa.indW1 = d1.indW; fa.indB1 = d1.indB; fa.indWr = d1.indWr; fa.indBr = d1.indBr;
  fa.indWo = h->indWo; fa.indBo = h->indBo; fa.indBp = h->indBp; fa.ldW0 = d0.ldW; fa.ldW1 = d1.ldW;
  fa.Y1 = d0.Y; fa.D1 = d0.D; fa.Dres1 = d0.Dres; fa.ldA0 = d0.ldA;
  fa.X2 = d1.X; fa.R2 = d1.Rr; fa.D2 = d1.D; fa.Dres2 = d1.Dres; fa.ldA1 = d1.ldA;
  fa.nLH = 2;
  if (h->fusedWideOk && h->nHidden == 3) {
    const DevHidden& d2 = h->hid[2];
    fa.nLH = 3; fa.indW2 = d2.indW; fa.indB2 = d2.indB; fa.indWr2 = d2.indWr; fa.indBr2 = d2.indBr; fa.ldW2 = d2.ldW; fa.resN2 = d2.resW;
    fa.X3 = d2.X; fa.R3 = d2.Rr; fa.D3 = d2.D; fa.Dres3 = d2.Dres; fa.ldA2 = d2.ldA;
  }
  fa.dOut = h->dOut; fa.ldDo = h->ldDo; fa.panelCtr = h->panelCtr; fa.Opart = h->panelOpart; fa.variant = h->dbgVariant; fa.xcdSafe = h->xcdSafe ? 1 : 0;
  for (int i = 0; i < h->dA; ++i) if (h->cfg.bounded[i]) fa.boundedMask |= 1ull << i;
  return fa;
}
int launchFused(hl_learner* h, int parity, hipStream_t s, bool nextSample = false, bool deferBeta = false, bool encodeCnt = false) {
  FusedArgs fa = fusedArgs(h, parity);
  ExtraArgs ex{}; const ExtraArgs* pex = nullptr;
  if (nextSample) { ex = extraSample(h, parity ^ 1, PH_A | PH_B); pex = &ex; }
  if (deferBeta) { fa.deferBeta = 1; ex.post = postArgs(h, parity ^ 1, POST_BETA); pex = &ex; }
  if (encodeCnt) { ex.post = postArgs(h, parity ^ 1, POST_ENCODE); pex = &ex; }
  HIPCK(timed(h, "fused_fwd_head_dx", s, [&] { return launch_fused(fa, h->Mmax, pex, s); }));
  return HL_OK;
}
HeadArgs headArgs(hl_learner* h, int parity);
int launchFusedWide(hl_learner* h, int parity, hipStream_t s, bool nextSample = false, bool deferBeta = false, bool encodeCnt = false) {
  FusedArgs fa = fusedArgs(h, parity);
  const HeadArgs ha = headArgs(h, parity);
  ExtraArgs ex{}; const ExtraArgs* pex = nullptr;
  if (nextSample) { ex = extraSample(h, parity ^ 1, PH_A | PH_B); pex = &ex; }
  if (deferBeta) { fa.deferBeta = 1; ex.post = postArgs(h, parity ^ 1, POST_BETA); pex = &ex; }
  if (encodeCnt) { ex.post = postArgs(h, parity ^ 1, POST_ENCODE); pex = &ex; }
  HIPCK(timed(h, "fused_wide", s, [&] { return launch_fused_wide(fa, ha, h->Mmax, pex, s); }));
  return HL_OK;
}
int launchFront(hl_learner* h, int parity, hipStream_t s, bool gather);
int launchStepChain(hl_learner* h, int parity, hipStream_t s, bool nextSample = false, bool wholeSampler = false, bool deferBeta = false, bool encodeCnt = false) {
  const AdamHyper hyp = adamHyper(h, parity);
  const StepBuf& sb = h->buf[parity];
  { const int rc = launchFront(h, parity, s, true); if (rc) return rc; }
  HeadArgs ha = headArgs(h, parity);
  ExtraArgs ex{}; const ExtraArgs* pex = nullptr;
  if (nextSample) { ex = extraSample(h, parity ^ 1, wholeSampler ? PH_ALL : (PH_A | PH_B)); pex = &ex; }
  if (deferBeta) { ha.deferBeta = 1; ex.post = postArgs(h, parity ^ 1, POST_BETA); pex = &ex; }
  if (encodeCnt) { ex.post = postArgs(h, parity ^ 1, POST_ENCODE); pex = &ex; }
  int fIdx[HL_MAX_HIDDEN], xIdx[HL_MAX_HIDDEN];
  for (int j = 0; j < h->nHidden; ++j) fIdx[j] = sb.fwdIdx[j];
  const int nX = (int)sb.dxIdx.size();
  for (int i = 0; i < nX; ++i) xIdx[i] = sb.dxIdx[i];
  HIPCK(timed(h, "step_chain", s, [&] { return launch_step_chain(h->dProbs, fIdx, h->nHidden, xIdx, nX, h->chainHT, h->Mmax, h->panelCtr, ha, h->sc, hyp, pex, s); }));
  return HL_OK;
}
ConvArgs convArgs(hl_learner* h, int parity);
int ensureConvPrep(hl_learner* h) {
  if (h->nConv == 0 || !h->convPrepStale) return HL_OK;
  const ConvArgs ca = convArgs(h, 0);
  HIPCK(launch_conv_prep(ca, h->stream));
  h->convPrepStale = false;
  return HL_OK;
}
ConvArgs convArgs(hl_learner* h, int parity) {
  ConvArgs ca{}; ca.sc = h->sc; ca.parity = parity; ca.B = h->convB; ca.nL = h->nConv;
  ca.W = h->W; ca.Wrw = h->W; ca.M1 = h->M1; ca.M2 = h->M2; ca.G = h->G;
  for (int l = 0; l < h->nConv; ++l) { ca.L[l] = h->cg[l]; ca.L[l].in = l == 0 ? h->buf[parity].X0 : h->cg[l - 1].Y; }
  return ca;
}
bool convFromReplay(const hl_learner* h) {
  if (h->nConv == 0 || !h->cg[0].rbRows || h->noConvReplay || h->extras > 0) return false;
  const ConvGeo& g = h->cg[0];
  return (h->dS & 3) == 0 && (g.InX & 3) == 0 && g.InC % (1 + h->nApp) == 0 && (long long)(g.InC / (1 + h->nApp)) * g.InY * g.InX == h->dS;
}
void convSource(hl_learner* h, int parity, ConvArgs* ca) {
  const DevBatch& bt = h->buf[parity].bt;
  ca->src.on = 1; ca->src.S = h->rp.S; ca->src.mean = h->rp.stMean; ca->src.scale = h->rp.stScale; ca->src.dS = h->dS; ca->src.nApp = h->nApp;
  ca->src.slot = bt.slot; ca->src.t = bt.t; ca->src.nextSrc = bt.nextSrc;
  ca->L[0].rbKind = (h->convRowsAtari && conv_rows_atari(ca->L[0], ca->src)) ? 1 : 0;
}
int launchFront(hl_learner* h, int parity, hipStream_t s, bool gather) {
  const StepBuf& sb = h->buf[parity];
  char nm[32];
  const bool windows = gather && h->recurrent && h->nConv > 0;
  DevBatch bt = sb.bt; DevScalars* sc = h->sc;
  if (windows) {
    WinRowsArgs wa{}; wa.sc = h->sc; wa.scW = h->scW; wa.slot = bt.slot; wa.t = bt.t; wa.nextSrc = bt.nextSrc; wa.B = h->B; wa.K = h->recK; wa.nBPTT = h->recWin - 1;
    wa.parity = parity; wa.slotW = h->winSlot; wa.tW = h->winT; wa.nextSrcW = h->winNextSrc;
    HIPCK(timed(h, "window_rows", s, [&] { return launch_window_rows(wa, s); }));
    bt.slot = h->winSlot; bt.t = h->winT; bt.nextSrc = h->winNextSrc; sc = h->scW;
  }
  const bool fromReplay = gather && convFromReplay(h);
  if (h->preproc && gather && !fromReplay) {
    StackGatherArgs ga{}; ga.sc = sc; ga.rp = h->rp; ga.bt = bt; ga.B = h->convB; ga.dS = h->dS; ga.nApp = h->nApp;
    ga.parity = parity; ga.X0 = sb.X0; ga.ldX0 = h->ldX0;
    HIPCK(timed(h, "stack_gather", s, [&] { return launch_stack_gather(ga, h->convMmax, s); }));
  }
  if (h->extras > 0)
    HIPCK(timed(h, "extras_copy", s, [&] { return launch_extras_copy(sc, parity, sb.X0, h->ldX0, h->dIn - h->extras, h->extras, h->hid[0].Y, h->hid[0].ldA, h->convMmax, s); }));
  if (h->nConv > 0) {
    ConvArgs ca = convArgs(h, parity);
    ca.sc = sc;
    if (fromReplay) { convSource(h, parity, &ca); ca.src.slot = bt.slot; ca.src.t = bt.t; ca.src.nextSrc = bt.nextSrc; }
    if (exchanging(h)) HIPCK(timed(h, "conv_prep", s, [&] { return launch_conv_prep(ca, s); }));
    else if (h->convPrepStale) return fail(h, HL_ERR_STATE, "convolution filter layouts are stale (ensureConvPrep was not called)");
    for (int l = 0; l < h->nConv; ++l) {
      snprintf(nm, sizeof(nm), "conv_fwd%d", l);
      if (l == 1 && h->convTail.atari) {
        HIPCK(timed(h, "conv_fwd_tail", s, [&] { return launch_conv_fwd_tail(ca, h->convTail, h->convMmax, s); }));
        break;
      }
      if (ca.L[l].rbRows) HIPCK(timed(h, nm, s, [&] { return launch_conv_forward_rows(ca, l, h->convMmax, s); }));
      else
      HIPCK(timed(h, nm, s, [&] { return launch_conv_forward(ca, l, h->convMmax, s); }));
    }
  }
  return HL_OK;
// ... 384 lines not shown
  h->preValid = false;
  if (h->sidePending) { HIPCK(hipStreamWaitEvent(h->stream, h->evSide, 0)); h->sidePending = false; }
  HIPCK(launch_rng_restore(h->sc, h->stream));
  return HL_OK;
}

int stepEager(hl_learner* h, const long long* dFlat) {
  hipStream_t s = h->stream;
  const long long k = h->nGradSteps + 1;
  const bool periodic = (k % 1000) == 0;
  const bool exch = exchanging(h);
  struct PushScope { hl_learner* h; ~PushScope() { h->pushGrad = false; } } pushScope{h};
  h->pushGrad = h->pushOk && h->xchg.on && !periodic;
  int p = 0, rc;
  if (h->preValid && !dFlat) {
    p = h->preParity; h->preValid = false;
    if (h->sidePending) { HIPCK(hipStreamWaitEvent(s, h->evSide, 0)); h->sidePending = false; }
  }
  else { rc = dropPresample(h); if (rc) return rc; rc = launchSample(h, 0, dFlat, true, s); if (rc) return rc; }
  const bool evict = evictionDue(h);
  if (h->bigBatch && !dFlat && !exch && !periodic && !evict && ((k + 1) % 1000) != 0 && h->cfg.dataSamplingAlgo == HL_SAMPLE_UNIFORM) {
    HIPCK(hipEventRecord(h->evMain, s)); HIPCK(hipStreamWaitEvent(h->sideStream, h->evMain, 0));
    SampleArgs sa = sampleArgs(h, p ^ 1, nullptr, false); sa.backupRng = 1;
    HIPCK(timed(h, "big_sample_ahead", h->sideStream, [&] { return launch_sample(sa, h->sideStream); }));
    HIPCK(hipEventRecord(h->evSide, h->sideStream));
    h->preValid = true; h->preParity = p ^ 1; h->sidePending = true;
  }
  rc = launchMlp(h, p, !exch, s); if (rc) return rc;
  h->lastParity = p;
  if (!periodic && !evict && !exch) return launchPost(h, p, POST_AGG | POST_BETA, s);
  rc = launchPost(h, p, POST_AGG, s); if (rc) return rc;
  if (periodic) {
    rc = launchPeriodicSweep(h); if (rc) return rc;
    rc = launchMoments(h); if (rc) return rc;
    rc = allreduceMoments(h); if (rc) return rc;
    if (oneBehind(h)) { rc = applyMomentsOneBehind(h); if (rc) return rc; }
    else { rc = launchMomentsApply(h, false, 10); if (rc) return rc; }
  }
  if (evict) { rc = applyRemoval(h); if (rc) return rc; rc = flushPending(h); if (rc) return rc; }
  if (exch) {
    if (wired(h)) { rc = launchPost(h, p, POST_ENCODE, s); if (rc) return rc; }
    if (h->xchg.on) return xchgAllreduce(h, h->G, (size_t)h->nParams + CNT_MSG_OFFSET + CNT_MSG_FLOATS, 0, p);
    rc = allreduceGrad(h); if (rc) return rc;
    rc = launchAdam(h, p); if (rc) return rc;
  }
  return launchPost(h, p, POST_BETA, s);
}

int captureSteps(hl_learner* h, int U, int p0, GraphSlot* slot, bool notify = false) {
  if (slot->exec) { hipGraphExecDestroy(slot->exec); slot->exec = nullptr; }
  if (slot->graph) { hipGraphDestroy(slot->graph); slot->graph = nullptr; }
  hipStream_t s0 = h->stream;
  HIPCK(hipStreamSynchronize(s0));
  if (h->bigBatch) { HIPCK(hipStreamSynchronize(h->sideStream)); h->sidePending = false; }
  HIPCK(hipStreamBeginCapture(s0, hipStreamCaptureModeThreadLocal));
  int rc = HL_OK;
  struct PushScope { hl_learner* h; ~PushScope() { h->pushGrad = false; } } pushScope{h};
  h->pushGrad = h->pushOk && h->xchg.on;
  const long long nColl0 = h->nCollectives;
  for (int j = 0; j < U && !rc; ++j) {
    const int p = (p0 + j) & 1;
    if (h->plainGraph) {
      SampleArgs sa = sampleArgs(h, p ^ 1, nullptr, false); sa.backupRng = 1;
      if (launch_sample(sa, s0) != hipSuccess) { rc = fail(h, HL_ERR_HIP, "sampler of the next step"); break; }
      rc = launchMlp(h, p, true, s0); if (rc) break;
      rc = launchPost(h, p, POST_AGG | POST_BETA, s0); if (rc) break;
      continue;
    }
    if (h->bigBatch) {
      if (hipEventRecord(h->evMain, s0) != hipSuccess || hipStreamWaitEvent(h->sideStream, h->evMain, 0) != hipSuccess) { rc = fail(h, HL_ERR_HIP, "fork of the sampler branch"); break; }
      SampleArgs sa = sampleArgs(h, p ^ 1, nullptr, false); sa.backupRng = 1;
      if (launch_sample(sa, h->sideStream) != hipSuccess || hipEventRecord(h->evSide, h->sideStream) != hipSuccess) { rc = fail(h, HL_ERR_HIP, "sampler branch"); break; }
      rc = launchMlp(h, p, true, s0); if (rc) break;
      rc = launchPost(h, p, POST_AGG | POST_BETA, s0); if (rc) break;
      if (hipStreamWaitEvent(s0, h->evSide, 0) != hipSuccess) { rc = fail(h, HL_ERR_HIP, "join of the sampler branch"); break; }
      continue;
    }
    const bool twoKernel = h->fusedOk || h->fusedWideOk || h->stepChainOk;
    if (twoKernel) {
      const bool single = !exchanging(h) && !h->noDeferBeta;
      const bool behind = oneBehind(h) && !h->noDeferBeta;
      const bool chainNarrow = h->stepChainOk && !exchanging(h) && !h->preproc && 2ll * h->B * h->dS <= 16384;
      const bool enc = behind && j > 0;
      rc = h->fusedOk ? launchFused(h, p, s0, true, single && j > 0, enc) : (h->fusedWideOk ? launchFusedWide(h, p, s0, true, single && j > 0, enc) : launchStepChain(h, p, s0, true, chainNarrow, single && j > 0, enc)); if (rc) break;
      if (chainNarrow) {
        rc = launchBackward(h, p, true, s0, true, POST_AGG | POST_BETA | (single && j + 1 < U ? POST_DEFER : 0), false, true); if (rc) break;
        continue;
      }
      if (!exchanging(h)) {
        rc = launchWeightGrad(h, p, true, s0, true, true, POST_AGG | POST_BETA | (single && j + 1 < U ? POST_DEFER : 0)); if (rc) break;
        continue;
      }
      rc = launchWeightGrad(h, p, false, s0, true, true, POST_AGG | (behind && j + 1 < U ? POST_DEFER : 0) | (enc ? POST_KEEPMSG : 0));
      if (!rc && h->xchg.on) { rc = xchgAllreduce(h, h->G, (size_t)h->nParams + CNT_MSG_OFFSET + CNT_MSG_FLOATS, 0, p); if (rc) break; continue; }
      if (!rc) rc = allreduceGrad(h);
      if (!rc) rc = launchAdam(h, p);
      if (!rc) rc = launchPost(h, p, POST_BETA, s0);
      if (rc) break;
      continue;
    }
    const bool exch = exchanging(h);
    if (h->recurrent) {
      const RecArgs ra = recArgs(h, p);
      const HeadArgs ha = headArgs(h, p);
      if (h->recFused && rec_step_fused_ok(ra, ha)) {
        const ExtraArgs exS = extraSample(h, p ^ 1, PH_A | PH_B);
        if (launch_rec_step_fused(ra, ha, &exS, s0) != hipSuccess) { rc = fail(h, HL_ERR_HIP, "rec_step_fused"); break; }
      } else {
        if (launch_rec_forward(ra, s0) != hipSuccess) { rc = fail(h, HL_ERR_HIP, "rec_forward"); break; }
        rc = launchHead(h, p, s0, true); if (rc) break;
        if (launch_rec_backward(ra, s0) != hipSuccess) { rc = fail(h, HL_ERR_HIP, "rec_backward"); break; }
      }
    } else {
      rc = launchForward(h, p, s0, true); if (rc) break;
      rc = launchHead(h, p, s0, true); if (rc) break;
    }
    rc = launchBackward(h, p, !exch, s0, true, exch ? POST_AGG : (POST_AGG | POST_BETA), h->recurrent); if (rc) break;
    if (exch) {
      if (h->xchg.on) { rc = xchgAllreduce(h, h->G, (size_t)h->nParams + CNT_MSG_OFFSET + CNT_MSG_FLOATS, 0, p); if (rc) break; continue; }
      rc = allreduceGrad(h);
      if (!rc) rc = launchAdam(h, p);
      if (!rc) rc = launchPost(h, p, POST_BETA, s0);
      if (rc) break;
    }
  }
  if (!rc && notify && launch_notify(h->sc, h->notifyPin, s0) != hipSuccess) rc = fail(h, HL_ERR_HIP, "notify");
  hipError_t e = hipStreamEndCapture(s0, &slot->graph);
  h->nCollectives = nColl0;
  if (rc) return rc;
  if (e != hipSuccess) return hipFail(h, e, "hipStreamEndCapture");
  HIPCK(hipGraphInstantiate(&slot->exec, slot->graph, nullptr, nullptr, 0));
  if (hipGraphUpload(slot->exec, s0) != hipSuccess) (void)hipGetLastError();
  slot->steps = U;
  return HL_OK;
}

void invalidateGraphs(hl_learner* h) {
  auto drop = [](GraphSlot& g) {
    if (g.exec) { hipGraphExecDestroy(g.exec); g.exec = nullptr; }
    if (g.graph) { hipGraphDestroy(g.graph); g.graph = nullptr; }
  };
  for (auto& gp : h->graphs) for (auto& g : gp) drop(g);
  for (auto& kv : h->exactGraphs) for (auto& g : kv.second) drop(g);
}

int touchReplay(hl_learner* h) {
  TouchArgs ta{}; const long long cap = h->capSlots, nE = (long long)h->order.size();
  auto add = [&](const void* p, long long bytes, int stride) { if (p && bytes > 0 && ta.n < 24) { ta.ptr[ta.n] = p; ta.bytes[ta.n] = bytes; ta.stride[ta.n] = stride; ++ta.n; } };
  add(h->rp.S, cap * h->dS * 4, 4096); add(h->rp.A, cap * h->dA * 8, 4096); add(h->rp.MU, cap * h->polDim * 8, 4096); add(h->rp.R, cap * 8, 4096);
  add(h->rp.V, cap * 4, 4096); add(h->rp.ADV, cap * 4, 4096); add(h->rp.RET, cap * 4, 4096); add(h->rp.DQ, cap * 4, 4096); add(h->rp.IMPW, cap * 4, 4096); add(h->rp.DKL, cap * 4, 4096);
  add(h->rp.posRec, (nE + 1) * (long long)sizeof(PosRec), 64); add(h->rp.posPrefix, (nE + 1) * 8, 64); add(h->rp.posEid, nE * 4, 64);
  add(h->rp.epAgg, (long long)h->nextEid * AGG_N * 4, 64); add(h->rp.epOff, (long long)h->nextEid * 8, 64); add(h->rp.epN, (long long)h->nextEid * 4, 64);
  add(h->rp.epTerm, (long long)h->nextEid, 64); add(h->rp.epTag, (long long)h->nextEid * 8, 64);
  add(h->W, h->nParams * 4, 64); add(h->M1, h->nParams * 4, 64); add(h->M2, h->nParams * 4, 64); add(h->G, h->nParams * 4, 64);
  ta.sink = h->G + h->nParams + 200;
  HIPCK(launch_touch(ta, h->stream));
  return HL_OK;
}

int prepareExact(hl_learner* h, int n) {
  if (!h->useGraph || n >= 1000 || (exchanging(h) && (!(h->exchGraph && wired(h)) || n > 64)) || h->cfg.dataSamplingAlgo != HL_SAMPLE_UNIFORM) return HL_OK;
  if (h->bigBatch && (n > 64 || exchanging(h))) return HL_OK;
  if (!graphUsable(h, n, 0)) return HL_OK;
  { const int rc = ensureConvPrep(h); if (rc) return rc; }
  if (!h->notifyPin) { HIPCK(hipHostMalloc((void**)&h->notifyPin, 64, hipHostMallocDefault)); *h->notifyPin = 0; }
  if (h->graphsStale) { invalidateGraphs(h); h->graphsStale = false; }
  if (h->exactGraphs.size() >= 8 && !h->exactGraphs.count(n)) {
    auto victim = h->exactGraphs.begin();
    for (auto& g : victim->second) { if (g.exec) hipGraphExecDestroy(g.exec); if (g.graph) hipGraphDestroy(g.graph); }
    h->exactGraphs.erase(victim);
  }
  auto& slots = h->exactGraphs[n];
  for (int p0 = 0; p0 < 2; ++p0) {
// ... 81 lines not shown
```

smarties_amd/csrc/tail_dev.h:

```cpp
#pragma once
#include "dev_common.h"

namespace hl {

#ifdef HL_TAIL_STAMPS
#define TSTAMP(sc, i) do { if (threadIdx.x == 0) (sc)->dbgT[i] = wall_clock64(); } while (0)
#define PSTAMP(sc, i) do { if (threadIdx.x == 0 && (a.mode & POST_DEFER)) (sc)->dbgT[i] = wall_clock64(); } while (0)
#else
#define TSTAMP(sc, i) do { } while (0)
#define PSTAMP(sc, i) do { } while (0)
#endif

#define SMAXB 1024
#define SMAXK (SMAXB / 256)

__device__ __forceinline__ void aggValues(float* ag, float oldV, float oldADV, float V, float Q) {
  const float oldQ = oldADV + oldV;
  ag[AGG_SUMQ2] += Q * Q - oldQ * oldQ;
  ag[AGG_SUMQ] += Q - oldQ;
  ag[AGG_MAXQ] = fmaxf(ag[AGG_MAXQ], Q);
  ag[AGG_MINQ] = fminf(ag[AGG_MINQ], Q);
}

__device__ __forceinline__ void encodeCounters(float* msg, const long long c4[4]) {
  for (int c = 0; c < 4; ++c) for (int q = 0; q < 4; ++q) msg[4 * c + q] = (float)((c4[c] >> (16 * q)) & 0xFFFF);
}

__device__ __forceinline__ void refEerPenal(DevScalars* sc, double fracOffPol, double learnRefer, double penalTol, double beta0, double alpha0, bool coherent) {
  const bool dec = fracOffPol > penalTol;
  const double beta = dec ? (1 - fmin(learnRefer, beta0)) * beta0
                          : (1 - fmin(learnRefer, beta0)) * beta0 + fmin(learnRefer, 1 - beta0);
  const bool decA = fabs(penalTol - fracOffPol) < 1e-3;
  const double alpha = decA ? (1 - fmin(learnRefer, alpha0)) * alpha0
                            : (1 - fmin(learnRefer, alpha0)) * alpha0 + fmin(learnRefer, 1 - alpha0);
  if (coherent) {
    __hip_atomic_store(&sc->beta, beta, __ATOMIC_RELAXED, __HIP_MEMORY_SCOPE_AGENT);
    __hip_atomic_store(&sc->alpha, alpha, __ATOMIC_RELAXED, __HIP_MEMORY_SCOPE_AGENT);
  } else { sc->beta = beta; sc->alpha = alpha; }
}

__device__ __forceinline__ void postPart(const PostArgs& a, long long* sFarDelta, unsigned* sMaxAbs, float* sFarP = nullptr, int farLdsFloats = 0) {
  const int mode = a.mode;
  DevScalars* sc = a.sc;
  const int tid = threadIdx.x, B = a.B;
  const double Cmax0 = sc->Cmax, Cinv0 = sc->Cinv, beta0 = sc->beta, alpha0 = sc->alpha;
  const double ema0 = sc->maxAbsErrEMA, bt1 = sc->adam_bt1, bt2 = sc->adam_bt2;
  const long long nGrad0 = sc->nGradSteps, nFarTot0 = sc->nFarTotal, nFarStat0 = sc->nFarStat;
  const long long nTrans = sc->nTransitions, cnt0 = sc->cnt[0], cnt1 = sc->cnt[1], cnt2 = sc->cnt[2], cnt3 = sc->cnt[3], nStep0 = sc->nStep, nEpL = sc->nEpisodes;
  const float maxAll0 = (mode & POST_AGG) ? sc->maxAbsErrAll : sc->maxAbsErrStep;
  PSTAMP(sc, 16);
  if (tid == 0) { *sFarDelta = 0; *sMaxAbs = 0u; }
  const int nEp = (int)nEpL, farPer = (nEp + 255) / 256;
  const bool defer = (mode & POST_DEFER) != 0;
  const int chunkMode = a.aggChunk;
  const bool farOn = (mode & POST_AGG) != 0, farLds = farOn && !defer && !chunkMode && sFarP && farPer <= FAR_REGS && FAR_REGS * 256 <= farLdsFloats;
  float farT[FAR_REGS], farL[FAR_REGS];
  unsigned long long farG0[FAR_SUB] = {};
  if (farLds) {
#pragma unroll
    for (int c = 0; c < FAR_SUB; ++c) farG0[c] = a.rp.farStart[c * 256 + tid];
#pragma unroll
    for (int i = 0; i < FAR_REGS; ++i) { farT[i] = a.rp.farP[i * 256 + tid]; farL[i] = a.rp.farN[i * 256 + tid]; }
  }
  if (!farLds) __syncthreads();
  PSTAMP(sc, 17);
  long long nFarStat = nFarStat0; float maxAll = maxAll0;
  if (mode & POST_AGG) {
    const float C = (float)Cmax0, invC = (float)Cinv0;
    const int bBeg = chunkMode == 1 ? (int)blockIdx.x * 256 : 0, bEnd = chunkMode == 1 ? min(B, bBeg + 256) : (chunkMode == 2 ? 0 : B);
    for (int b0 = bBeg; b0 < bEnd; b0 += 256) {
      const int b = b0 + tid;
      const bool in = b < B;
      const int e = in ? a.bt.pEid[b] : -1;
      const int ePrev = (in && b > 0) ? a.bt.pEid[b - 1] : -2;
      const int eNext = (in && b + 1 < B) ? a.bt.pEid[b + 1] : -3;
      const int nxt0 = in ? a.bt.pNextOf[b] : -1;
      float Q0 = 0, E0 = 0, D0 = 0, W0 = 0, V0 = 0, oW0 = 0, oE0 = 0, oD0 = 0, oV0 = 0, oA0 = 0, Vn0 = 0, oNV0 = 0, oNA0 = 0;
      if (in) {
        E0 = a.bt.newDQ[b]; D0 = a.bt.newDKL[b]; W0 = a.bt.newW[b]; V0 = a.bt.newV[b];
        oW0 = a.bt.oldW[b]; oE0 = a.bt.oldDQ[b]; oD0 = a.bt.oldDKL[b]; oV0 = a.bt.oldV[b]; oA0 = a.bt.oldADV[b];
        Vn0 = a.bt.nextV[b]; oNV0 = a.bt.oldNextV[b]; oNA0 = a.bt.oldNextADV[b];
        Q0 = a.hasAdv ? a.bt.newQ[b] : V0;
      }
      f32x4 s0 = {0.f, 0.f, 0.f, 0.f}, s1 = s0, s2 = s0;
      if (in && a.aggStaged) {
        const f32x4* st = reinterpret_cast<const f32x4*>(a.bt.aggIn + (size_t)b * AGG_N);
        s0 = st[0]; s1 = st[1]; s2 = st[2];
      }
      const bool leader = in && ePrev != e;
      float myMaxAbs = 0.f;
      if (b0 == 0 && farLds) {
#pragma unroll
        for (int i = 0; i < FAR_REGS; ++i) sFarP[i * 256 + tid] = farT[i];
        __syncthreads();
      }
      if (leader) {
      float* ag = a.rp.epAgg + (size_t)e * AGG_N;
      float g[AGG_N]; float Nf;
      if (a.aggStaged) {
        g[0] = s0[0]; g[1] = s0[1]; g[2] = s0[2]; g[3] = s0[3]; g[4] = s1[0]; g[5] = s1[1]; g[6] = s1[2]; g[7] = s1[3];
        g[8] = s2[0]; g[9] = 0.f; g[10] = 0.f; g[11] = 0.f; Nf = s2[1];
      } else {
        Nf = (float)a.rp.epN[e];
#pragma unroll
        for (int q = 0; q < AGG_N; ++q) g[q] = ag[q];
      }
      const float invN = 1 / Nf;
      int j = b; bool more = true;
      float Qf = Q0, E = E0, D = D0, W = W0, Vf = V0, oW = oW0, oE = oE0, oD = oD0, oV = oV0, oA = oA0, Vn = Vn0, oNV = oNV0, oNA = oNA0;
      int nxt = nxt0;
      while (more) {
        if (nxt >= 0) aggValues(g, oNV, oNA, Vn, Vn);
        const float wasFar = (oW > C || oW < invC) ? 1.f : 0.f;
        const float isFar = (W > C || W < invC) ? 1.f : 0.f;
        g[AGG_AVGKL] += invN * (D - oD);
        g[AGG_FRACFAR] += invN * (isFar - wasFar);
        g[AGG_AVGSQERR] += invN * (E * E - oE * oE);
        g[AGG_MAXABSERR] = fmaxf(g[AGG_MAXABSERR], fabsf(E));
        aggValues(g, oV, oA, Vf, Qf);
        const int en = (j == b) ? eNext : ((j + 1 < B) ? a.bt.pEid[j + 1] : -3);
        more = (en == e);
        if (more) {
          ++j;
          nxt = a.bt.pNextOf[j];
          E = a.bt.newDQ[j]; D = a.bt.newDKL[j]; W = a.bt.newW[j]; Vf = a.bt.newV[j];
          oW = a.bt.oldW[j]; oE = a.bt.oldDQ[j]; oD = a.bt.oldDKL[j]; oV = a.bt.oldV[j]; oA = a.bt.oldADV[j];
          Vn = a.bt.nextV[j]; oNV = a.bt.oldNextV[j]; oNA = a.bt.oldNextADV[j];
          Qf = a.hasAdv ? a.bt.newQ[j] : Vf;
        }
      }
#pragma unroll
      for (int q = 0; q < AGG_N; ++q) ag[q] = g[q];
      if (farOn) {
        const int pos = a.bt.pos[b], t = pos / farPer, idx = (pos - t * farPer) * 256 + t;
        a.rp.farP[idx] = g[AGG_FRACFAR];
        if (farLds) sFarP[idx] = g[AGG_FRACFAR];
      }
      myMaxAbs = fmaxf(g[AGG_MAXABSERR], 0.f);
      }
      for (int o = 32; o > 0; o >>= 1) myMaxAbs = fmaxf(myMaxAbs, __shfl_xor(myMaxAbs, o, 64));
      if ((tid & 63) == 0) { if (chunkMode == 1) atomicMax(&sc->maxAbsScratch, __float_as_uint(myMaxAbs)); else atomicMax(sMaxAbs, __float_as_uint(myMaxAbs)); }
    }
    if (chunkMode == 1) return;
    if (chunkMode == 2 && tid == 0) { *sMaxAbs = sc->maxAbsScratch; sc->maxAbsScratch = 0u; }
    PSTAMP(sc, 18);
    __syncthreads();
    PSTAMP(sc, 19);
    unsigned long long* sScan = reinterpret_cast<unsigned long long*>(sFarDelta) + 2;
    const int farCnt = farSegment(nEp, farPer);
    const float* const gFarP = a.rp.farP; const float* const gFarN = a.rp.farN;
    unsigned long long* const gFarStart = a.rp.farStart;
    long long farTotal = nFarTot0;
    if (defer) {
    } else if (farLds) {
#pragma unroll
      for (int i = 0; i < FAR_REGS; ++i) farT[i] = sFarP[i * 256 + tid];
      TSTAMP(sc, 14);
      unsigned long long tot = 0;
      if (!farCountRegs(farT, farL, farG0, gFarStart, reinterpret_cast<unsigned*>(sScan), &tot)) tot = farCountMem<false>(sFarP, gFarN, farCnt, gFarStart, sScan);
#ifdef HL_TAIL_STAMPS
      if (tid == 0 && (long long)(tot >> 48) > sc->dbgT[12]) sc->dbgT[12] = (long long)(tot >> 48);
      tot &= 0xffffffffffffull;
#endif
      farTotal = (long long)tot;
      TSTAMP(sc, 15);
    } else {
      __threadfence();
      farTotal = (long long)farCountMem<true>(gFarP, gFarN, farCnt, gFarStart, sScan);
    }
    if (tid == 0) {
      long long nFarTot = farTotal;
      maxAll = fmaxf(maxAll0, __uint_as_float(*sMaxAbs));
      const double Cm = 1 + a.clipImpWeight / (1 + (double)(nGrad0 + 1) * a.epsAnneal);
      if (Cm <= 1) nFarTot = 0;
      nFarStat = nFarTot;
      sc->maxAbsErrAll = maxAll; sc->maxAbsErrStep = maxAll; sc->Cmax = Cm; sc->Cinv = 1 / Cm; sc->cnt[3] = nTrans;
      if (!defer) { sc->nFarTotal = nFarTot; sc->nFarStat = nFarStat; sc->cnt[2] = nFarStat; }
      if (a.nRanks > 1) { sc->cnt[0] = sc->seenLocal[0]; sc->cnt[1] = sc->seenLocal[1]; }
      if (a.cntMsg && !(mode & POST_KEEPMSG)) {
        if (a.behind) { const long long c4[4] = {sc->cntPrev[0], sc->cntPrev[1], sc->cntPrev[2], sc->cntPrev[3]}; encodeCounters(a.cntMsg, c4); }
        else {
        const long long c4[4] = {sc->seenLocal[0], sc->seenLocal[1], nFarStat, nTrans};
        encodeCounters(a.cntMsg, c4);
        }
      }
    }
  }
  if ((mode & POST_ENCODE) && a.cntMsg && tid == 0) {
    if (a.behind) { const long long c4[4] = {sc->cntPrev[0], sc->cntPrev[1], sc->cntPrev[2], sc->cntPrev[3]}; encodeCounters(a.cntMsg, c4); }
    else {
    const long long c4[4] = {sc->seenLocal[0], sc->seenLocal[1], sc->cnt[2], sc->cnt[3]};
    encodeCounters(a.cntMsg, c4);
    }
  }
  if ((mode & (POST_BETA | POST_INIT)) && tid == 0) {
    const bool rewritten = (mode & POST_AGG) && a.nRanks > 1;
    long long cntR[4] = {rewritten ? sc->cnt[0] : cnt0, rewritten ? sc->cnt[1] : cnt1, cnt2, cnt3};
    if (a.cntMsg && (mode & POST_BETA)) {
      for (int c = 0; c < 4; ++c) {
        long long v = 0;
        for (int q = 0; q < 4; ++q) v += (long long)(a.cntMsg[4 * c + q] + 0.5f) << (16 * q);
        cntR[c] = v; sc->cnt[c] = v;
      }
    }
    sc->seenUpd[0] = cntR[0]; sc->seenUpd[1] = cntR[1];
    const long long nFar = a.nRanks > 1 ? cntR[2] : nFarStat;
    const long long nStored = a.nRanks > 1 ? cntR[3] : nTrans;
    const double fracOffPol = (double)nFar / (double)(nStored > 1 ? nStored : 1);
    const double nDataSize = fmax(a.maxObsGlobal, (double)nStored);
    const double learnRefer = 0.1 * a.batchGlobal / nDataSize;
    if (!defer) refEerPenal(sc, fracOffPol, learnRefer, a.penalTol, beta0, alpha0, false);
    if (mode & POST_BETA) {
      const double lrLoc = 0.1 * a.batchGlobal / fmax(a.maxObsGlobal, (double)nTrans);
      sc->maxAbsErrEMA = ema0 + lrLoc * ((double)maxAll - ema0);
      double nb1 = bt1 * 0.9; if (nb1 < (double)FLT_EPSILON) nb1 = 0;
      double nb2 = bt2 * 0.999; if (nb2 < (double)FLT_EPSILON) nb2 = 0;
      sc->adam_bt1 = nb1; sc->adam_bt2 = nb2;
      sc->nStep = nStep0 + 1;
      sc->nGradSteps = nGrad0 + 1;
      sc->etaEff[a.parity ^ 1] = adamEtaEff(nStep0 + 1, nb1, nb2, a.eta0, a.epsAnneal);
      if (a.behind) { sc->cntPrev[0] = sc->seenLocal[0]; sc->cntPrev[1] = sc->seenLocal[1]; sc->cntPrev[2] = nFarStat; sc->cntPrev[3] = nTrans; }
    }
  }
  PSTAMP(sc, 20);
}

__device__ __forceinline__ unsigned mtTemper(unsigned z) {
  z ^= (z >> 11); z ^= (z << 7) & 0x9d2c5680u; z ^= (z << 15) & 0xefc60000u; z ^= (z >> 18);
  return z;
}
__device__ __forceinline__ unsigned mtF(unsigned a, unsigned b) {
  const unsigned y = (a & 0x80000000u) | (b & 0x7fffffffu);
  return (y >> 1) ^ ((y & 1u) ? 0x9908b0dfu : 0u);
}
__device__ void mtTwist(unsigned* x, unsigned* xo) {
  const int tid = threadIdx.x;
  for (int k = tid; k < 624; k += 256) xo[k] = x[k];
  __syncthreads();
  if (tid < 227) x[tid] = xo[tid + 397] ^ mtF(xo[tid], xo[tid + 1]);
  __syncthreads();
  if (tid < 227) x[227 + tid] = x[tid] ^ mtF(xo[227 + tid], xo[228 + tid]);
  __syncthreads();
  if (tid < 169) x[454 + tid] = x[227 + tid] ^ mtF(xo[454 + tid], xo[455 + tid]);
  __syncthreads();
  if (tid == 0) x[623] = x[396] ^ mtF(xo[623], x[0]);
  __syncthreads();
}
__device__ void mtDraw(unsigned* x, unsigned* xo, int* pPos, unsigned* raw, int n) {
  int done = 0;
  while (done < n) {
    int pos = *pPos;
    __syncthreads();
    if (pos >= 624) { mtTwist(x, xo); pos = 0; }
    const int take = min(n - done, 624 - pos);
    for (int i = threadIdx.x; i < take; i += 256) raw[done + i] = mtTemper(x[pos + i]);
    if (threadIdx.x == 0) *pPos = pos + take;
    __syncthreads();
    done += take;
  }
}

__device__ __forceinline__ int scanRows(int K, const bool* flag, int* excl, int* sWave ) {
  const int tid = threadIdx.x, lane = tid & 63, wave = tid >> 6;
  int base = 0;
  _Pragma("unroll") for (int r = 0; r < SMAXK; ++r) if (r < K) {
    const unsigned long long m = __ballot(flag[r]);
    const int within = __popcll(m & ((1ull << lane) - 1ull));
    if (lane == 0) sWave[wave] = __popcll(m);
    __syncthreads();
    const int w0 = sWave[0], w1 = sWave[1], w2 = sWave[2], w3 = sWave[3];
    excl[r] = base + within + (wave > 0 ? w0 : 0) + (wave > 1 ? w1 : 0) + (wave > 2 ? w2 : 0);
    base += w0 + w1 + w2 + w3;
    __syncthreads();
  }
  return base;
}

__device__ __forceinline__ unsigned cmpx(unsigned key, unsigned other, bool lower, bool up) {
  const unsigned mn = min(key, other), mx = max(key, other);
  return (lower == up) ? mn : mx;
}
__device__ void waveLocalRounds(unsigned* vals, int Bp, int k, int jStart) {
  const int lane = threadIdx.x & 63, wave = threadIdx.x >> 6;
  for (int blk = wave; blk * 64 < Bp; blk += 4) {
    const int i = blk * 64 + lane;
    unsigned key = vals[i];
    if (k <= 64) {
      for (int kk = 2; kk <= k; kk <<= 1)
        for (int j = kk >> 1; j > 0; j >>= 1)
          key = cmpx(key, (unsigned)__shfl_xor((int)key, j, 64), (i & j) == 0, (i & kk) == 0);
    } else {
      for (int j = jStart; j > 0; j >>= 1)
        key = cmpx(key, (unsigned)__shfl_xor((int)key, j, 64), (i & j) == 0, (i & k) == 0);
    }
    vals[i] = key;
  }
}
__device__ void bitonicSort(unsigned* vals, int Bp) {
  __syncthreads();
  waveLocalRounds(vals, Bp, 64, 32);
  for (int k = 128; k <= Bp; k <<= 1) {
    for (int j = k >> 1; j >= 64; j >>= 1) {
      __syncthreads();
// ... 250 lines not shown
        const PosRec rec = findPosition(a.rp, f, nEp, nData, &lo);
        const int t = (int)(f - rec.prefix);
        sSlot[b] = rec.off + t;
        hasNext[r] = (t + 2 == rec.N && !(rec.eidTerm < 0));
      }
    }
    scanRows(K, hasNext, nextIdx, sWave);
    _Pragma("unroll") for (int r = 0; r < SMAXK; ++r) if (r < K) { const int b = r * 256 + tid; if (b < B) sNextRow[b] = hasNext[r] ? B + nextIdx[r] : -1; }
    __syncthreads();
    if (part == 0) TSTAMP(sc, 22);
    const int per = (B + nParts - 1) / nParts, b0 = part * per, b1 = min(B, b0 + per);
    const int total = max(0, b1 - b0) * dS;
    constexpr int GU = 4;
    for (int e0 = tid; e0 < total; e0 += 256 * GU) {
      float sv[GU], sn[GU]; int bb[GU], ii[GU], nr[GU];
#pragma unroll
      for (int u = 0; u < GU; ++u) {
        const int e = e0 + 256 * u;
        bb[u] = -1; sv[u] = 0.f; sn[u] = 0.f; ii[u] = 0; nr[u] = -1;
        if (e < total) {
          const int b = b0 + e / dS; bb[u] = b; ii[u] = e - (b - b0) * dS;
          const long long sl = sSlot[b];
          sv[u] = a.rp.S[(size_t)sl * dS + ii[u]];
          nr[u] = sNextRow[b];
          if (nr[u] >= 0) sn[u] = a.rp.S[(size_t)(sl + 1) * dS + ii[u]];
        }
      }
#pragma unroll
      for (int u = 0; u < GU; ++u) if (bb[u] >= 0) {
        const float mu = sMean[ii[u]], scl = sScale[ii[u]];
        a.X0[(size_t)bb[u] * a.ldX0 + ii[u]] = (sv[u] - mu) * scl;
        if (nr[u] >= 0) a.X0[(size_t)nr[u] * a.ldX0 + ii[u]] = (sn[u] - mu) * scl;
      }
    }
    if (part == 0) TSTAMP(sc, 23);
    return;
  }
  if (tid == 0) {
    const long long want = a.tagSeq ? -sc->sampleSeq : sc->nStep + 1;
    int spins = 0;
    while (__hip_atomic_load(sc->gatherFlag + a.parity, __ATOMIC_RELAXED, __HIP_MEMORY_SCOPE_AGENT) != want) {
      __builtin_amdgcn_s_sleep(2);
      if (++spins > (1 << 22)) { sc->errFlag = 78; break; }
    }
  }
  __syncthreads();
  if (part == 0) TSTAMP(sc, 22);
  const int per = (B + nParts - 1) / nParts, b0 = part * per, b1 = min(B, b0 + per);
  const int total = max(0, b1 - b0) * dS;
  constexpr int GU = 4;
  for (int e0 = tid; e0 < total; e0 += 256 * GU) {
    float sv[GU], sn[GU]; int bb[GU], ii[GU], nr[GU]; long long sl[GU];
#pragma unroll
    for (int u = 0; u < GU; ++u) {
      const int e = e0 + 256 * u;
      bb[u] = -1; nr[u] = -1; sl[u] = 0; ii[u] = 0;
      if (e < total) {
        const int b = b0 + e / dS; bb[u] = b; ii[u] = e - (b - b0) * dS;
        sl[u] = __hip_atomic_load(a.bt.slot + b, __ATOMIC_RELAXED, __HIP_MEMORY_SCOPE_AGENT);
        nr[u] = __hip_atomic_load(a.bt.nextOf + b, __ATOMIC_RELAXED, __HIP_MEMORY_SCOPE_AGENT);
      }
    }
#pragma unroll
    for (int u = 0; u < GU; ++u) {
      sv[u] = 0.f; sn[u] = 0.f;
      if (bb[u] >= 0) {
        sv[u] = a.rp.S[(size_t)sl[u] * dS + ii[u]];
        if (nr[u] >= 0) sn[u] = a.rp.S[(size_t)(sl[u] + 1) * dS + ii[u]];
      }
    }
#pragma unroll
    for (int u = 0; u < GU; ++u) if (bb[u] >= 0) {
      const float mu = sMean[ii[u]], scl = sScale[ii[u]];
      a.X0[(size_t)bb[u] * a.ldX0 + ii[u]] = (sv[u] - mu) * scl;
      if (nr[u] >= 0) a.X0[(size_t)nr[u] * a.ldX0 + ii[u]] = (sn[u] - mu) * scl;
    }
  }
  if (part == 0) TSTAMP(sc, 23);
}

__device__ __forceinline__ void postPhase(const PostArgs& a, unsigned char* smem) {
  long long* sFarDelta = reinterpret_cast<long long*>(smem);
  unsigned* sMaxAbs = reinterpret_cast<unsigned*>(smem + 8);
  postPart(a, sFarDelta, sMaxAbs, reinterpret_cast<float*>(smem + 64), (TAIL_LDS_BYTES - 64) / 4);
}

__device__ __forceinline__ void farBetaPhase(const PostArgs& a, unsigned char* smem) {
  DevScalars* sc = a.sc;
  const int tid = threadIdx.x;
  TSTAMP(sc, 10);
  const double Cmax = sc->Cmax, beta0 = sc->beta, alpha0 = sc->alpha;
  const long long nTrans = sc->nTransitions, nEpL = sc->nEpisodes, nGrad = sc->nGradSteps;
  const int nEp = (int)nEpL, per = (nEp + 255) / 256;
  unsigned long long* sScan = reinterpret_cast<unsigned long long*>(smem);
  const float* const gFarP = a.rp.farP; const float* const gFarN = a.rp.farN; unsigned long long* const gFarStart = a.rp.farStart;
  unsigned long long tot = 0;
  bool done = false;
  if (per <= FAR_REGS) {
    float f[FAR_REGS], l[FAR_REGS]; unsigned long long g0[FAR_SUB];
#pragma unroll
    for (int c = 0; c < FAR_SUB; ++c) g0[c] = gFarStart[c * 256 + tid];
#pragma unroll
    for (int i = 0; i < FAR_REGS; ++i) { f[i] = gFarP[i * 256 + tid]; l[i] = gFarN[i * 256 + tid]; }
    done = farCountRegs(f, l, g0, gFarStart, reinterpret_cast<unsigned*>(sScan), &tot);
#ifdef HL_TAIL_STAMPS
    if (tid == 0 && (long long)(tot >> 48) > sc->dbgT[12]) sc->dbgT[12] = (long long)(tot >> 48);
    tot &= 0xffffffffffffull;
#endif
  }
  if (!done) tot = farCountMem<false>(gFarP, gFarN, farSegment(nEp, per), gFarStart, sScan);
  TSTAMP(sc, 11);
  if (tid != 0) return;
  const long long nFar = Cmax <= 1 ? 0 : (long long)tot;
  sc->nFarTotal = nFar; sc->nFarStat = nFar; sc->cnt[2] = nFar;
  if (a.mode & POST_ENCODE) {
    const long long c4[4] = {sc->seenLocal[0], sc->seenLocal[1], nFar, nTrans};
    encodeCounters(a.cntMsg, c4);
    return;
  }
  const double fracOffPol = (double)nFar / (double)(nTrans > 1 ? nTrans : 1);
  const double learnRefer = 0.1 * a.batchGlobal / fmax(a.maxObsGlobal, (double)nTrans);
  refEerPenal(sc, fracOffPol, learnRefer, a.penalTol, beta0, alpha0, true);
  __builtin_amdgcn_s_waitcnt(0);
  __hip_atomic_store(&sc->betaSeq, nGrad, __ATOMIC_RELAXED, __HIP_MEMORY_SCOPE_AGENT);
}

__device__ __forceinline__ void runExtra(const ExtraArgs& ex, unsigned char* smem) {
  if (ex.role == 1) samplePhases(ex.samp, ex.phases, smem);
  else if (ex.role == 2) postPhase(ex.post, smem);
  else if (ex.role == 3) farBetaPhase(ex.post, smem);
}

}
```

Measured before the change: 14.87 million transitions/s.

## Defer per-episode aggregate update into next fused kernel's side block

Moves the per-episode statistics aggregation (epAgg update, far-policy fraction patch, max-abs-error EMA) out of the weight-grad tail. In single-replica fused mode, the tail now only advances scalars, and a spare block of the next step's fused forward kernel does the aggregation. That block also recounts far-policy transitions for beta. The fused kernel no longer prefetches epAgg into registers or stages aggIn, which cuts global loads and register pressure on the critical path. In exchange, the aggregate runs one step late on a single block, and the far count must be patched before counting.

```diff
diff --git a/smarties_amd/csrc/fused.hip b/smarties_amd/csrc/fused.hip
--- a/smarties_amd/csrc/fused.hip
+++ b/smarties_amd/csrc/fused.hip
@@ -119,7 +119,7 @@
   if (blockIdx.x < 8) {
     if (threadIdx.x >= 256) return;
     if (blockIdx.x == 0) { if (extra.role == 1) { samplePhases(extra.samp, extra.phases, smem); FEND(22); } }
-    else if (blockIdx.x == 1 && (a.deferBeta || extra.post.mode == POST_ENCODE)) { farBetaPhase(extra.post, smem); if (threadIdx.x == 0) a.sc->dbgT[23] = wall_clock64(); }
+    else if (blockIdx.x == 1 && (a.deferBeta || extra.post.mode == POST_ENCODE)) { deferredPhase(extra.post, smem); if (threadIdx.x == 0) a.sc->dbgT[23] = wall_clock64(); }
     else if (extra.role == 1 && (extra.phases & PH_PUBLISH)) gatherHelper(extra.samp, blockIdx.x - 1, 7, smem);
     return;
   }
@@ -201,8 +201,6 @@
   const bool rowValid = eth && row < nRows, isNext = rowValid && row >= B;
   int bSrc = 0; long long slot = 0;
   if (rowValid) { bSrc = isNext ? a.bt.nextSrc[row - B] : row; slot = a.bt.slot[bSrc]; }
-  int eidv = 0;
-  if (rowValid && !isNext) eidv = a.bt.eid[row];
   float sv[QS];
 #pragma unroll
   for (int q = 0; q < QS; ++q) {
@@ -256,8 +254,6 @@
     const int f = tid + NT * q; w1r[q] = z4;
     if (f < 16 * H4) { const int r = f / H4, c4 = f % H4; w1r[q] = *reinterpret_cast<const f32x4*>(W1 + (size_t)(n0 + r) * a.ldW1 + 4 * c4); }
   }
-  const bool aggOwner = ((em & (HT - 1)) == n) && rowValid && !isNext && en < AGG_N;
-
   double act = 0, bMean = 0, bStd = 1; float misc = 0.f;
   if (rowValid && !isNext && en < dA) {
     act = a.rp.A[(size_t)slot * dA + en];
@@ -268,12 +264,6 @@
     if (!isNext) arr = en == 0 ? a.rp.RET : en == 1 ? a.rp.DQ : en == 2 ? a.rp.DKL : en == 3 ? a.rp.IMPW : en == 4 ? a.rp.V : en == 5 ? a.rp.ADV : nullptr;
     else { arr = en == 6 ? a.rp.V : en == 7 ? a.rp.ADV : nullptr; sl = slot + 1; }
     if (arr) misc = arr[sl];
-  }
-
-  float aggv = 0.f;
-  if constexpr (CHAIN) {
-    asm volatile("" : "+v"(eidv));
-    if (aggOwner) aggv = en < AGG_USED ? a.rp.epAgg[(size_t)eidv * AGG_N + en] : (en == AGG_LEN ? (float)a.rp.epN[eidv] : 0.f);
   }
 
   const bool live = rowValid && !isNext;
@@ -347,8 +337,6 @@
   FSTAMP(2);
   FVARIANT_STOP(2);
   if (eth && row < B) a.Y1[(size_t)row * ldA0 + n0 + en] = y1o;
-  asm volatile("" : "+v"(eidv));
-  if (aggOwner) aggv = en < AGG_USED ? a.rp.epAgg[(size_t)eidv * AGG_N + en] : (en == AGG_LEN ? (float)a.rp.epN[eidv] : 0.f);
   }
   constexpr bool SPLITW = (NW == 8 && H >= 16);
   constexpr int XW = CHAIN ? CW : (SPLITW ? 4 : KWAVES);
@@ -702,7 +690,6 @@
   }
   __syncthreads();
   FSTAMP(12);
-  if (((em & (HT - 1)) == n) && rowValid && !isNext && en < AGG_N) a.bt.aggIn[(size_t)bSrc * AGG_N + en] = aggv;
   if (eth && row < B) {
     const float v = redSum<KWAVES>(red, tid);
     float dres = v;
diff --git a/smarties_amd/csrc/fusedw.hip b/smarties_amd/csrc/fusedw.hip
--- a/smarties_amd/csrc/fusedw.hip
+++ b/smarties_amd/csrc/fusedw.hip
@@ -65,7 +65,7 @@
   if (blockIdx.x < 8) {
     if (threadIdx.x >= 256) return;
     if (blockIdx.x == 0) { if (extra.role == 1) samplePhases(extra.samp, extra.phases, smem); }
-    else if (blockIdx.x == 1 && (a.deferBeta || extra.post.mode == POST_ENCODE)) farBetaPhase(extra.post, smem);
+    else if (blockIdx.x == 1 && (a.deferBeta || extra.post.mode == POST_ENCODE)) deferredPhase(extra.post, smem);
     return;
   }
   constexpr int NT = FW_NT, NW = NT / 64, HT = H / 16, H4 = H / 4;
diff --git a/smarties_amd/csrc/hl_types.h b/smarties_amd/csrc/hl_types.h
--- a/smarties_amd/csrc/hl_types.h
+++ b/smarties_amd/csrc/hl_types.h
@@ -37,6 +37,7 @@
   long long dbgT[32];
   long long dbgStep[128];
   long long cntPrev[4];
+  float aggC, aggInvC;
 };
 
 struct PosRec {
@@ -68,7 +69,7 @@
   float* farP; float* farN; unsigned long long* farStart;
 };
 enum { AGG_TOTR = 0, AGG_AVGKL, AGG_FRACFAR, AGG_AVGSQERR, AGG_MAXABSERR, AGG_SUMQ2, AGG_SUMQ,
-       AGG_MAXQ, AGG_MINQ, AGG_USED, AGG_LEN = 9 , AGG_N = 12 };
+       AGG_MAXQ, AGG_MINQ, AGG_USED, AGG_N = 12 };
 
 struct DevBatch {
   long long* flat;
@@ -90,7 +91,6 @@
   float *oldDQ, *oldDKL, *oldW, *oldV, *oldADV;
   float *nextV, *oldNextV, *oldNextADV;
   float* gParam;
-  float* aggIn;
 };
 
 struct DevHidden {
diff --git a/smarties_amd/csrc/kernels.h b/smarties_amd/csrc/kernels.h
--- a/smarties_amd/csrc/kernels.h
+++ b/smarties_amd/csrc/kernels.h
@@ -166,7 +166,6 @@
   int nRanks;
   int parity;
   float eta0;
-  int aggStaged;
   int hasAdv;
   int aggChunk;
   float* cntMsg;
@@ -174,7 +173,8 @@
 };
 enum { POST_AGG = 1, POST_BETA = 2, POST_INIT = 4, POST_ENCODE = 8 ,
        POST_DEFER = 16 ,
-       POST_KEEPMSG = 32  };
+       POST_KEEPMSG = 32 ,
+       POST_DEFER_AGG = 64  };
 
 struct AdamArgs {
   const DevScalars* sc; float* W; float* M1; float* M2; const float* G; long long n;
diff --git a/smarties_amd/csrc/learner.cpp b/smarties_amd/csrc/learner.cpp
--- a/smarties_amd/csrc/learner.cpp
+++ b/smarties_amd/csrc/learner.cpp
@@ -329,7 +329,6 @@
     HIPCK(devAlloc(&bt.oldDQ, B)); HIPCK(devAlloc(&bt.oldDKL, B)); HIPCK(devAlloc(&bt.oldW, B)); HIPCK(devAlloc(&bt.oldV, B));
     HIPCK(devAlloc(&bt.oldADV, B)); HIPCK(devAlloc(&bt.nextV, B)); HIPCK(devAlloc(&bt.oldNextV, B));
     HIPCK(devAlloc(&bt.oldNextADV, B)); HIPCK(devAlloc(&bt.gParam, (size_t)B * std::max(h->nSig, 1)));
-    HIPCK(devAlloc(&bt.aggIn, (size_t)B * AGG_N));
   }
   HIPCK(devAlloc(&h->dFlatGiven, B));
   HIPCK(devAlloc(&h->dMoments, (size_t)2 * h->dS + 3)); HIPCK(devAlloc(&h->dMomentsPrev, (size_t)2 * h->dS + 3)); HIPCK(devAlloc(&h->dStatsOut, 16)); HIPCK(devAlloc(&h->dStatsIns, 16));
@@ -384,7 +383,7 @@
     DevBatch& bt = h->buf[pb].bt;
     void* bp[] = {h->buf[pb].X0, bt.sVals, bt.tag, bt.pEid, bt.pNextOf, bt.flat, bt.pos, bt.eid, bt.t, bt.slot, bt.nextOf, bt.nextSrc,
       bt.O, bt.G, bt.rho, bt.dkl, bt.dq, bt.far, bt.newDQ, bt.newDKL, bt.newW, bt.newV, bt.newQ, bt.oldDQ, bt.oldDKL, bt.oldW,
-      bt.oldV, bt.oldADV, bt.nextV, bt.oldNextV, bt.oldNextADV, bt.gParam, bt.aggIn};
+      bt.oldV, bt.oldADV, bt.nextV, bt.oldNextV, bt.oldNextADV, bt.gParam};
     for (void* q : bp) if (q) hipFree(q);
   }
   for (void* q : {(void*)h->segY, (void*)h->segDres, (void*)h->segScratch}) if (q) hipFree(q);
diff --git a/smarties_amd/csrc/step_exec.h b/smarties_amd/csrc/step_exec.h
--- a/smarties_amd/csrc/step_exec.h
+++ b/smarties_amd/csrc/step_exec.h
@@ -216,7 +216,7 @@
   PostArgs pa{}; pa.sc = h->sc; pa.rp = h->rp; pa.bt = h->buf[parity].bt; pa.B = h->B; pa.mode = mode;
   pa.clipImpWeight = h->cfg.clipImpWeight; pa.epsAnneal = h->cfg.epsAnneal; pa.penalTol = h->cfg.penalTol;
   pa.maxObsGlobal = (double)h->maxObsGlobal; pa.batchGlobal = (double)h->Bglobal; pa.nRanks = exchanging(h) ? 2 : 1;
-  pa.parity = parity; pa.eta0 = (float)h->cfg.learnrate; pa.aggStaged = h->fusedOk ? 1 : 0; pa.hasAdv = h->nAdv > 0 ? 1 : 0;
+  pa.parity = parity; pa.eta0 = (float)h->cfg.learnrate; pa.hasAdv = h->nAdv > 0 ? 1 : 0;
   pa.cntMsg = wired(h) ? h->G + h->nParams + CNT_MSG_OFFSET : nullptr;
   pa.behind = oneBehind(h) ? 1 : 0;
   return pa;
@@ -288,22 +288,22 @@
   for (int i = 0; i < h->dA; ++i) if (h->cfg.bounded[i]) fa.boundedMask |= 1ull << i;
   return fa;
 }
-int launchFused(hl_learner* h, int parity, hipStream_t s, bool nextSample = false, bool deferBeta = false, bool encodeCnt = false) {
+int launchFused(hl_learner* h, int parity, hipStream_t s, bool nextSample = false, bool deferBeta = false, bool encodeCnt = false, bool deferAgg = false) {
   FusedArgs fa = fusedArgs(h, parity);
   ExtraArgs ex{}; const ExtraArgs* pex = nullptr;
   if (nextSample) { ex = extraSample(h, parity ^ 1, PH_A | PH_B); pex = &ex; }
-  if (deferBeta) { fa.deferBeta = 1; ex.post = postArgs(h, parity ^ 1, POST_BETA); pex = &ex; }
+  if (deferBeta) { fa.deferBeta = 1; ex.post = postArgs(h, parity ^ 1, POST_BETA | (deferAgg ? POST_DEFER_AGG : 0)); pex = &ex; }
   if (encodeCnt) { ex.post = postArgs(h, parity ^ 1, POST_ENCODE); pex = &ex; }
   HIPCK(timed(h, "fused_fwd_head_dx", s, [&] { return launch_fused(fa, h->Mmax, pex, s); }));
   return HL_OK;
 }
 HeadArgs headArgs(hl_learner* h, int parity);
-int launchFusedWide(hl_learner* h, int parity, hipStream_t s, bool nextSample = false, bool deferBeta = false, bool encodeCnt = false) {
+int launchFusedWide(hl_learner* h, int parity, hipStream_t s, bool nextSample = false, bool deferBeta = false, bool encodeCnt = false, bool deferAgg = false) {
   FusedArgs fa = fusedArgs(h, parity);
   const HeadArgs ha = headArgs(h, parity);
   ExtraArgs ex{}; const ExtraArgs* pex = nullptr;
   if (nextSample) { ex = extraSample(h, parity ^ 1, PH_A | PH_B); pex = &ex; }
-  if (deferBeta) { fa.deferBeta = 1; ex.post = postArgs(h, parity ^ 1, POST_BETA); pex = &ex; }
+  if (deferBeta) { fa.deferBeta = 1; ex.post = postArgs(h, parity ^ 1, POST_BETA | (deferAgg ? POST_DEFER_AGG : 0)); pex = &ex; }
   if (encodeCnt) { ex.post = postArgs(h, parity ^ 1, POST_ENCODE); pex = &ex; }
   HIPCK(timed(h, "fused_wide", s, [&] { return launch_fused_wide(fa, ha, h->Mmax, pex, s); }));
   return HL_OK;
@@ -854,13 +854,14 @@
       const bool behind = oneBehind(h) && !h->noDeferBeta;
       const bool chainNarrow = h->stepChainOk && !exchanging(h) && !h->preproc && 2ll * h->B * h->dS <= 16384;
       const bool enc = behind && j > 0;
-      rc = h->fusedOk ? launchFused(h, p, s0, true, single && j > 0, enc) : (h->fusedWideOk ? launchFusedWide(h, p, s0, true, single && j > 0, enc) : launchStepChain(h, p, s0, true, chainNarrow, single && j > 0, enc)); if (rc) break;
+      const bool aggToo = single && (h->fusedOk || h->fusedWideOk) && !wired(h);
+      rc = h->fusedOk ? launchFused(h, p, s0, true, single && j > 0, enc, aggToo) : (h->fusedWideOk ? launchFusedWide(h, p, s0, true, single && j > 0, enc, aggToo) : launchStepChain(h, p, s0, true, chainNarrow, single && j > 0, enc)); if (rc) break;
       if (chainNarrow) {
         rc = launchBackward(h, p, true, s0, true, POST_AGG | POST_BETA | (single && j + 1 < U ? POST_DEFER : 0), false, true); if (rc) break;
         continue;
       }
       if (!exchanging(h)) {
-        rc = launchWeightGrad(h, p, true, s0, true, true, POST_AGG | POST_BETA | (single && j + 1 < U ? POST_DEFER : 0)); if (rc) break;
+        rc = launchWeightGrad(h, p, true, s0, true, true, POST_AGG | POST_BETA | (single && j + 1 < U ? POST_DEFER | (aggToo ? POST_DEFER_AGG : 0) : 0)); if (rc) break;
         continue;
       }
       rc = launchWeightGrad(h, p, false, s0, true, true, POST_AGG | (behind && j + 1 < U ? POST_DEFER : 0) | (enc ? POST_KEEPMSG : 0));
diff --git a/smarties_amd/csrc/tail_dev.h b/smarties_amd/csrc/tail_dev.h
--- a/smarties_amd/csrc/tail_dev.h
+++ b/smarties_amd/csrc/tail_dev.h
@@ -37,6 +37,104 @@
     __hip_atomic_store(&sc->beta, beta, __ATOMIC_RELAXED, __HIP_MEMORY_SCOPE_AGENT);
     __hip_atomic_store(&sc->alpha, alpha, __ATOMIC_RELAXED, __HIP_MEMORY_SCOPE_AGENT);
   } else { sc->beta = beta; sc->alpha = alpha; }
+}
+
+struct AggRow { int e, ePrev, eNext, nxt, pos; float Q, E, D, W, V, oW, oE, oD, oV, oA, Vn, oNV, oNA; };
+__device__ __forceinline__ int farIndex(int pos, int farPer) { const int t = pos / farPer; return (pos - t * farPer) * 256 + t; }
+__device__ __forceinline__ AggRow aggLoadRow(const PostArgs& a, int b, bool in) {
+  AggRow r{};
+  r.e = in ? a.bt.pEid[b] : -1;
+  r.ePrev = (in && b > 0) ? a.bt.pEid[b - 1] : -2;
+  r.eNext = (in && b + 1 < a.B) ? a.bt.pEid[b + 1] : -3;
+  r.nxt = in ? a.bt.pNextOf[b] : -1;
+  r.pos = in ? a.bt.pos[b] : 0;
+  if (in) {
+    r.E = a.bt.newDQ[b]; r.D = a.bt.newDKL[b]; r.W = a.bt.newW[b]; r.V = a.bt.newV[b];
+    r.oW = a.bt.oldW[b]; r.oE = a.bt.oldDQ[b]; r.oD = a.bt.oldDKL[b]; r.oV = a.bt.oldV[b]; r.oA = a.bt.oldADV[b];
+    r.Vn = a.bt.nextV[b]; r.oNV = a.bt.oldNextV[b]; r.oNA = a.bt.oldNextADV[b];
+    r.Q = a.hasAdv ? a.bt.newQ[b] : r.V;
+  }
+  return r;
+}
+__device__ __forceinline__ float aggLeaderRun(const PostArgs& a, int b, const AggRow& r, float C, float invC, int farPer, float* sFarP) {
+  const int e = r.e, B = a.B;
+  float* ag = a.rp.epAgg + (size_t)e * AGG_N;
+  float g[AGG_N];
+  const float Nf = (float)a.rp.epN[e];
+#pragma unroll
+  for (int q = 0; q < AGG_N; ++q) g[q] = ag[q];
+  const float invN = 1 / Nf;
+  int j = b; bool more = true;
+  float Qf = r.Q, E = r.E, D = r.D, W = r.W, Vf = r.V, oW = r.oW, oE = r.oE, oD = r.oD, oV = r.oV, oA = r.oA, Vn = r.Vn, oNV = r.oNV, oNA = r.oNA;
+  int nxt = r.nxt;
+  while (more) {
+    if (nxt >= 0) aggValues(g, oNV, oNA, Vn, Vn);
+    const float wasFar = (oW > C || oW < invC) ? 1.f : 0.f;
+    const float isFar = (W > C || W < invC) ? 1.f : 0.f;
+    g[AGG_AVGKL] += invN * (D - oD);
+    g[AGG_FRACFAR] += invN * (isFar - wasFar);
+    g[AGG_AVGSQERR] += invN * (E * E - oE * oE);
+    g[AGG_MAXABSERR] = fmaxf(g[AGG_MAXABSERR], fabsf(E));
+    aggValues(g, oV, oA, Vf, Qf);
+    const int en = (j == b) ? r.eNext : ((j + 1 < B) ? a.bt.pEid[j + 1] : -3);
+    more = (en == e);
+    if (more) {
+      ++j;
+      nxt = a.bt.pNextOf[j];
+      E = a.bt.newDQ[j]; D = a.bt.newDKL[j]; W = a.bt.newW[j]; Vf = a.bt.newV[j];
+      oW = a.bt.oldW[j]; oE = a.bt.oldDQ[j]; oD = a.bt.oldDKL[j]; oV = a.bt.oldV[j]; oA = a.bt.oldADV[j];
+      Vn = a.bt.nextV[j]; oNV = a.bt.oldNextV[j]; oNA = a.bt.oldNextADV[j];
+      Qf = a.hasAdv ? a.bt.newQ[j] : Vf;
+    }
+  }
+#pragma unroll
+  for (int q = 0; q < AGG_N; ++q) ag[q] = g[q];
+  const int idx = farIndex(r.pos, farPer);
+  a.rp.farP[idx] = g[AGG_FRACFAR];
+  if (sFarP) sFarP[idx] = g[AGG_FRACFAR];
+  return fmaxf(g[AGG_MAXABSERR], 0.f);
+}
+
+__device__ __forceinline__ float farPatchRun(const PostArgs& a, int b, const AggRow& r, float C, float invC, float frac, float Nf) {
+  const int e = r.e, B = a.B;
+  const float invN = 1 / Nf;
+  int j = b; bool more = true;
+  float W = r.W, oW = r.oW;
+  while (more) {
+    const float wasFar = (oW > C || oW < invC) ? 1.f : 0.f;
+    const float isFar = (W > C || W < invC) ? 1.f : 0.f;
+    frac += invN * (isFar - wasFar);
+    const int en = (j == b) ? r.eNext : ((j + 1 < B) ? a.bt.pEid[j + 1] : -3);
+    more = (en == e);
+    if (more) { ++j; W = a.bt.newW[j]; oW = a.bt.oldW[j]; }
+  }
+  return frac;
+}
+
+__device__ __forceinline__ double clipAnneal(const PostArgs& a, long long nGrad0) { return 1 + a.clipImpWeight / (1 + (double)(nGrad0 + 1) * a.epsAnneal); }
+__device__ __forceinline__ double maxErrEma(const PostArgs& a, double ema0, float maxAll, long long nTrans) {
+  const double lrLoc = 0.1 * a.batchGlobal / fmax(a.maxObsGlobal, (double)nTrans);
+  return ema0 + lrLoc * ((double)maxAll - ema0);
+}
+__device__ __forceinline__ void advanceStep(DevScalars* sc, const PostArgs& a, long long nStep0, long long nGrad0, double bt1, double bt2) {
+  double nb1 = bt1 * 0.9; if (nb1 < (double)FLT_EPSILON) nb1 = 0;
+  double nb2 = bt2 * 0.999; if (nb2 < (double)FLT_EPSILON) nb2 = 0;
+  sc->adam_bt1 = nb1; sc->adam_bt2 = nb2;
+  sc->nStep = nStep0 + 1;
+  sc->nGradSteps = nGrad0 + 1;
+  sc->etaEff[a.parity ^ 1] = adamEtaEff(nStep0 + 1, nb1, nb2, a.eta0, a.epsAnneal);
+}
+
+__device__ __forceinline__ void postScalars(const PostArgs& a) {
+  if (threadIdx.x != 0) return;
+  DevScalars* sc = a.sc;
+  const double Cmax0 = sc->Cmax, Cinv0 = sc->Cinv, bt1 = sc->adam_bt1, bt2 = sc->adam_bt2;
+  const long long nGrad0 = sc->nGradSteps, nStep0 = sc->nStep, nTrans = sc->nTransitions, cnt0 = sc->cnt[0], cnt1 = sc->cnt[1];
+  const double Cm = clipAnneal(a, nGrad0);
+  sc->aggC = (float)Cmax0; sc->aggInvC = (float)Cinv0;
+  sc->Cmax = Cm; sc->Cinv = 1 / Cm; sc->cnt[3] = nTrans;
+  sc->seenUpd[0] = cnt0; sc->seenUpd[1] = cnt1;
+  advanceStep(sc, a, nStep0, nGrad0, bt1, bt2);
 }
 
 __device__ __forceinline__ void postPart(const PostArgs& a, long long* sFarDelta, unsigned* sMaxAbs, float* sFarP = nullptr, int farLdsFloats = 0) {
@@ -71,73 +169,14 @@
     for (int b0 = bBeg; b0 < bEnd; b0 += 256) {
       const int b = b0 + tid;
       const bool in = b < B;
-      const int e = in ? a.bt.pEid[b] : -1;
-      const int ePrev = (in && b > 0) ? a.bt.pEid[b - 1] : -2;
-      const int eNext = (in && b + 1 < B) ? a.bt.pEid[b + 1] : -3;
-      const int nxt0 = in ? a.bt.pNextOf[b] : -1;
-      float Q0 = 0, E0 = 0, D0 = 0, W0 = 0, V0 = 0, oW0 = 0, oE0 = 0, oD0 = 0, oV0 = 0, oA0 = 0, Vn0 = 0, oNV0 = 0, oNA0 = 0;
-      if (in) {
-        E0 = a.bt.newDQ[b]; D0 = a.bt.newDKL[b]; W0 = a.bt.newW[b]; V0 = a.bt.newV[b];
-        oW0 = a.bt.oldW[b]; oE0 = a.bt.oldDQ[b]; oD0 = a.bt.oldDKL[b]; oV0 = a.bt.oldV[b]; oA0 = a.bt.oldADV[b];
-        Vn0 = a.bt.nextV[b]; oNV0 = a.bt.oldNextV[b]; oNA0 = a.bt.oldNextADV[b];
-        Q0 = a.hasAdv ? a.bt.newQ[b] : V0;
-      }
-      f32x4 s0 = {0.f, 0.f, 0.f, 0.f}, s1 = s0, s2 = s0;
-      if (in && a.aggStaged) {
-        const f32x4* st = reinterpret_cast<const f32x4*>(a.bt.aggIn + (size_t)b * AGG_N);
-        s0 = st[0]; s1 = st[1]; s2 = st[2];
-      }
-      const bool leader = in && ePrev != e;
-      float myMaxAbs = 0.f;
+      const AggRow r = aggLoadRow(a, b, in);
       if (b0 == 0 && farLds) {
 #pragma unroll
         for (int i = 0; i < FAR_REGS; ++i) sFarP[i * 256 + tid] = farT[i];
         __syncthreads();
       }
-      if (leader) {
-      float* ag = a.rp.epAgg + (size_t)e * AGG_N;
-      float g[AGG_N]; float Nf;
-      if (a.aggStaged) {
-        g[0] = s0[0]; g[1] = s0[1]; g[2] = s0[2]; g[3] = s0[3]; g[4] = s1[0]; g[5] = s1[1]; g[6] = s1[2]; g[7] = s1[3];
-        g[8] = s2[0]; g[9] = 0.f; g[10] = 0.f; g[11] = 0.f; Nf = s2[1];
-      } else {
-        Nf = (float)a.rp.epN[e];
-#pragma unroll
-        for (int q = 0; q < AGG_N; ++q) g[q] = ag[q];
-      }
-      const float invN = 1 / Nf;
-      int j = b; bool more = true;
-      float Qf = Q0, E = E0, D = D0, W = W0, Vf = V0, oW = oW0, oE = oE0, oD = oD0, oV = oV0, oA = oA0, Vn = Vn0, oNV = oNV0, oNA = oNA0;
-      int nxt = nxt0;
-      while (more) {
-        if (nxt >= 0) aggValues(g, oNV, oNA, Vn, Vn);
-        const float wasFar = (oW > C || oW < invC) ? 1.f : 0.f;
-        const float isFar = (W > C || W < invC) ? 1.f : 0.f;
-        g[AGG_AVGKL] += invN * (D - oD);
-        g[AGG_FRACFAR] += invN * (isFar - wasFar);
-        g[AGG_AVGSQERR] += invN * (E * E - oE * oE);
-        g[AGG_MAXABSERR] = fmaxf(g[AGG_MAXABSERR], fabsf(E));
-        aggValues(g, oV, oA, Vf, Qf);
-        const int en = (j == b) ? eNext : ((j + 1 < B) ? a.bt.pEid[j + 1] : -3);
-        more = (en == e);
-        if (more) {
-          ++j;
-          nxt = a.bt.pNextOf[j];
-          E = a.bt.newDQ[j]; D = a.bt.newDKL[j]; W = a.bt.newW[j]; Vf = a.bt.newV[j];
-          oW = a.bt.oldW[j]; oE = a.bt.oldDQ[j]; oD = a.bt.oldDKL[j]; oV = a.bt.oldV[j]; oA = a.bt.oldADV[j];
-          Vn = a.bt.nextV[j]; oNV = a.bt.oldNextV[j]; oNA = a.bt.oldNextADV[j];
-          Qf = a.hasAdv ? a.bt.newQ[j] : Vf;
-        }
-      }
-#pragma unroll
-      for (int q = 0; q < AGG_N; ++q) ag[q] = g[q];
-      if (farOn) {
-        const int pos = a.bt.pos[b], t = pos / farPer, idx = (pos - t * farPer) * 256 + t;
-        a.rp.farP[idx] = g[AGG_FRACFAR];
-        if (farLds) sFarP[idx] = g[AGG_FRACFAR];
-      }
-      myMaxAbs = fmaxf(g[AGG_MAXABSERR], 0.f);
-      }
+      float myMaxAbs = 0.f;
+      if (in && r.ePrev != r.e) myMaxAbs = aggLeaderRun(a, b, r, C, invC, farPer, farLds ? sFarP : nullptr);
       for (int o = 32; o > 0; o >>= 1) myMaxAbs = fmaxf(myMaxAbs, __shfl_xor(myMaxAbs, o, 64));
       if ((tid & 63) == 0) { if (chunkMode == 1) atomicMax(&sc->maxAbsScratch, __float_as_uint(myMaxAbs)); else atomicMax(sMaxAbs, __float_as_uint(myMaxAbs)); }
     }
@@ -171,7 +210,7 @@
     if (tid == 0) {
       long long nFarTot = farTotal;
       maxAll = fmaxf(maxAll0, __uint_as_float(*sMaxAbs));
-      const double Cm = 1 + a.clipImpWeight / (1 + (double)(nGrad0 + 1) * a.epsAnneal);
+      const double Cm = clipAnneal(a, nGrad0);
       if (Cm <= 1) nFarTot = 0;
       nFarStat = nFarTot;
       sc->maxAbsErrAll = maxAll; sc->maxAbsErrStep = maxAll; sc->Cmax = Cm; sc->Cinv = 1 / Cm; sc->cnt[3] = nTrans;
@@ -211,14 +250,8 @@
     const double learnRefer = 0.1 * a.batchGlobal / nDataSize;
     if (!defer) refEerPenal(sc, fracOffPol, learnRefer, a.penalTol, beta0, alpha0, false);
     if (mode & POST_BETA) {
-      const double lrLoc = 0.1 * a.batchGlobal / fmax(a.maxObsGlobal, (double)nTrans);
-      sc->maxAbsErrEMA = ema0 + lrLoc * ((double)maxAll - ema0);
-      double nb1 = bt1 * 0.9; if (nb1 < (double)FLT_EPSILON) nb1 = 0;
-      double nb2 = bt2 * 0.999; if (nb2 < (double)FLT_EPSILON) nb2 = 0;
-      sc->adam_bt1 = nb1; sc->adam_bt2 = nb2;
-      sc->nStep = nStep0 + 1;
-      sc->nGradSteps = nGrad0 + 1;
-      sc->etaEff[a.parity ^ 1] = adamEtaEff(nStep0 + 1, nb1, nb2, a.eta0, a.epsAnneal);
+      sc->maxAbsErrEMA = maxErrEma(a, ema0, maxAll, nTrans);
+      advanceStep(sc, a, nStep0, nGrad0, bt1, bt2);
       if (a.behind) { sc->cntPrev[0] = sc->seenLocal[0]; sc->cntPrev[1] = sc->seenLocal[1]; sc->cntPrev[2] = nFarStat; sc->cntPrev[3] = nTrans; }
     }
   }
@@ -635,47 +668,121 @@
 __device__ __forceinline__ void postPhase(const PostArgs& a, unsigned char* smem) {
   long long* sFarDelta = reinterpret_cast<long long*>(smem);
   unsigned* sMaxAbs = reinterpret_cast<unsigned*>(smem + 8);
+  if (a.mode & POST_DEFER_AGG) { postScalars(a); return; }
   postPart(a, sFarDelta, sMaxAbs, reinterpret_cast<float*>(smem + 64), (TAIL_LDS_BYTES - 64) / 4);
 }
 
-__device__ __forceinline__ void farBetaPhase(const PostArgs& a, unsigned char* smem) {
+struct FarIn { double Cmax, beta0, alpha0; long long nTrans, nGrad; int nEp, per; float l[FAR_REGS]; unsigned long long g0[FAR_SUB]; };
+__device__ __forceinline__ void farLoad(const PostArgs& a, FarIn& in) {
+  const DevScalars* sc = a.sc;
+  const int tid = threadIdx.x;
+  in.Cmax = sc->Cmax; in.beta0 = sc->beta; in.alpha0 = sc->alpha;
+  in.nTrans = sc->nTransitions; in.nGrad = sc->nGradSteps;
+  in.nEp = (int)sc->nEpisodes; in.per = (in.nEp + 255) / 256;
+  if (in.per <= FAR_REGS) {
+#pragma unroll
+    for (int c = 0; c < FAR_SUB; ++c) in.g0[c] = a.rp.farStart[c * 256 + tid];
+#pragma unroll
+    for (int i = 0; i < FAR_REGS; ++i) in.l[i] = a.rp.farN[i * 256 + tid];
+  }
+}
+__device__ __forceinline__ void farCountBeta(const PostArgs& a, unsigned char* smem, const FarIn& in, const float (&f)[FAR_REGS], const float* sFarP, bool patched) {
   DevScalars* sc = a.sc;
   const int tid = threadIdx.x;
-  TSTAMP(sc, 10);
-  const double Cmax = sc->Cmax, beta0 = sc->beta, alpha0 = sc->alpha;
-  const long long nTrans = sc->nTransitions, nEpL = sc->nEpisodes, nGrad = sc->nGradSteps;
-  const int nEp = (int)nEpL, per = (nEp + 255) / 256;
   unsigned long long* sScan = reinterpret_cast<unsigned long long*>(smem);
   const float* const gFarP = a.rp.farP; const float* const gFarN = a.rp.farN; unsigned long long* const gFarStart = a.rp.farStart;
   unsigned long long tot = 0;
   bool done = false;
-  if (per <= FAR_REGS) {
-    float f[FAR_REGS], l[FAR_REGS]; unsigned long long g0[FAR_SUB];
-#pragma unroll
-    for (int c = 0; c < FAR_SUB; ++c) g0[c] = gFarStart[c * 256 + tid];
-#pragma unroll
-    for (int i = 0; i < FAR_REGS; ++i) { f[i] = gFarP[i * 256 + tid]; l[i] = gFarN[i * 256 + tid]; }
-    done = farCountRegs(f, l, g0, gFarStart, reinterpret_cast<unsigned*>(sScan), &tot);
+  if (in.per <= FAR_REGS) {
+    done = farCountRegs(f, in.l, in.g0, gFarStart, reinterpret_cast<unsigned*>(sScan), &tot);
 #ifdef HL_TAIL_STAMPS
     if (tid == 0 && (long long)(tot >> 48) > sc->dbgT[12]) sc->dbgT[12] = (long long)(tot >> 48);
     tot &= 0xffffffffffffull;
 #endif
   }
-  if (!done) tot = farCountMem<false>(gFarP, gFarN, farSegment(nEp, per), gFarStart, sScan);
+  if (!done) {
+    const int cnt = farSegment(in.nEp, in.per);
+    if (sFarP) tot = farCountMem<false>(sFarP, gFarN, cnt, gFarStart, sScan);
+    else if (patched) tot = farCountMem<true>(gFarP, gFarN, cnt, gFarStart, sScan);
+    else tot = farCountMem<false>(gFarP, gFarN, cnt, gFarStart, sScan);
+  }
   TSTAMP(sc, 11);
   if (tid != 0) return;
-  const long long nFar = Cmax <= 1 ? 0 : (long long)tot;
+  const long long nFar = in.Cmax <= 1 ? 0 : (long long)tot;
   sc->nFarTotal = nFar; sc->nFarStat = nFar; sc->cnt[2] = nFar;
   if (a.mode & POST_ENCODE) {
-    const long long c4[4] = {sc->seenLocal[0], sc->seenLocal[1], nFar, nTrans};
+    const long long c4[4] = {sc->seenLocal[0], sc->seenLocal[1], nFar, in.nTrans};
     encodeCounters(a.cntMsg, c4);
     return;
   }
-  const double fracOffPol = (double)nFar / (double)(nTrans > 1 ? nTrans : 1);
-  const double learnRefer = 0.1 * a.batchGlobal / fmax(a.maxObsGlobal, (double)nTrans);
-  refEerPenal(sc, fracOffPol, learnRefer, a.penalTol, beta0, alpha0, true);
+  const double fracOffPol = (double)nFar / (double)(in.nTrans > 1 ? in.nTrans : 1);
+  const double learnRefer = 0.1 * a.batchGlobal / fmax(a.maxObsGlobal, (double)in.nTrans);
+  refEerPenal(sc, fracOffPol, learnRefer, a.penalTol, in.beta0, in.alpha0, true);
   __builtin_amdgcn_s_waitcnt(0);
-  __hip_atomic_store(&sc->betaSeq, nGrad, __ATOMIC_RELAXED, __HIP_MEMORY_SCOPE_AGENT);
+  __hip_atomic_store(&sc->betaSeq, in.nGrad, __ATOMIC_RELAXED, __HIP_MEMORY_SCOPE_AGENT);
+}
+__device__ __forceinline__ void farBetaPhase(const PostArgs& a, unsigned char* smem) {
+  TSTAMP(a.sc, 10);
+  FarIn in; farLoad(a, in);
+  float f[FAR_REGS];
+#pragma unroll
+  for (int i = 0; i < FAR_REGS; ++i) f[i] = in.per <= FAR_REGS ? a.rp.farP[i * 256 + threadIdx.x] : 0.f;
+  farCountBeta(a, smem, in, f, nullptr, false);
+}
+
+__device__ __forceinline__ void aggBetaPhase(const PostArgs& a, unsigned char* smem) {
+  DevScalars* sc = a.sc;
+  const int tid = threadIdx.x, B = a.B;
+  const float C = sc->aggC, invC = sc->aggInvC, maxAll0 = sc->maxAbsErrAll;
+  const double ema0 = sc->maxAbsErrEMA;
+  FarIn in; farLoad(a, in);
+  const int farPer = in.per;
+  const bool farLds = farPer <= FAR_REGS;
+  unsigned* sMaxAbs = reinterpret_cast<unsigned*>(smem + 48);
+  float* sFarP = farLds ? reinterpret_cast<float*>(smem + 64) : nullptr;
+  if (tid == 0) *sMaxAbs = 0u;
+  const AggRow r0 = aggLoadRow(a, tid, tid < B);
+  const bool lead0 = tid < B && r0.ePrev != r0.e;
+  const int idx0 = farIndex(r0.pos, farPer);
+  const float Nf0 = lead0 ? a.rp.farN[idx0] : 1.f, frac0 = (lead0 && !farLds) ? a.rp.farP[idx0] : 0.f;
+  if (farLds) {
+#pragma unroll
+    for (int i = 0; i < FAR_REGS; ++i) sFarP[i * 256 + tid] = a.rp.farP[i * 256 + tid];
+  }
+  __syncthreads();
+  for (int b0 = 0; b0 < B; b0 += 256) {
+    const int b = b0 + tid;
+    const AggRow r = b0 == 0 ? r0 : aggLoadRow(a, b, b < B);
+    if (b < B && r.ePrev != r.e) {
+      const int idx = b0 == 0 ? idx0 : farIndex(r.pos, farPer);
+      const float Nf = b0 == 0 ? Nf0 : a.rp.farN[idx];
+      if (farLds) sFarP[idx] = farPatchRun(a, b, r, C, invC, sFarP[idx], Nf);
+      else a.rp.farP[idx] = farPatchRun(a, b, r, C, invC, b0 == 0 ? frac0 : a.rp.farP[idx], Nf);
+    }
+  }
+  if (!farLds) __threadfence();
+  __syncthreads();
+  float f[FAR_REGS];
+#pragma unroll
+  for (int i = 0; i < FAR_REGS; ++i) f[i] = farLds ? sFarP[i * 256 + tid] : 0.f;
+  farCountBeta(a, smem, in, f, sFarP, !farLds);
+  for (int b0 = 0; b0 < B; b0 += 256) {
+    const int b = b0 + tid;
+    const AggRow r = b0 == 0 ? r0 : aggLoadRow(a, b, b < B);
+    float myMaxAbs = 0.f;
+    if (b < B && r.ePrev != r.e) myMaxAbs = aggLeaderRun(a, b, r, C, invC, farPer, nullptr);
+    for (int o = 32; o > 0; o >>= 1) myMaxAbs = fmaxf(myMaxAbs, __shfl_xor(myMaxAbs, o, 64));
+    if ((tid & 63) == 0) atomicMax(sMaxAbs, __float_as_uint(myMaxAbs));
+  }
+  __syncthreads();
+  if (tid == 0) {
+    const float maxAll = fmaxf(maxAll0, __uint_as_float(*sMaxAbs));
+    sc->maxAbsErrAll = maxAll; sc->maxAbsErrStep = maxAll;
+    sc->maxAbsErrEMA = maxErrEma(a, ema0, maxAll, in.nTrans);
+  }
+}
+__device__ __forceinline__ void deferredPhase(const PostArgs& a, unsigned char* smem) {
+  if (a.mode & POST_DEFER_AGG) aggBetaPhase(a, smem); else farBetaPhase(a, smem);
 }
 
 __device__ __forceinline__ void runExtra(const ExtraArgs& ex, unsigned char* smem) {
```

Result: slower. 13.78 million transitions/s (-7.4%).
